# zhang-xuan1314/ABC-Net

Hardware: NVIDIA B200
Metric: images_per_sec_unet_fwd_decode (higher is better)
Workload: dtype bf16

## Files before the change

abcnet_b200/_lib.py:

```python
from __future__ import annotations

import ctypes as C
import os

_HERE = os.path.dirname(os.path.abspath(__file__))
LIB_PATH = os.path.join(_HERE, "libabcnet_b200.so")

EXPORTS = (
    "abc_last_error", "abc_version", "abc_device_ok", "abc_sm_count", "abc_launch_count",
    "abc_conv3x3_c1", "abc_conv3x3_c1_u8", "abc_conv3x3_cn", "abc_conv3x3_cn_wgrad", "abc_conv3x3_stem", "abc_conv_igemm", "abc_conv_wpack_bytes", "abc_decode_peaks",
    "abc_loss_partials", "abc_loss_backward", "abc_loss_partials_p8",
    "abc_bn_stats", "abc_bn_finalize", "abc_bn_act", "abc_bn_act_backward", "abc_nchw_to_p8", "abc_channel_sum",
    "abc_nchw_to_p8_ex", "abc_deinterleave2", "abc_conv_wgrad", "abc_conv3x3_c1_wgrad", "abc_conv3x3_c1_raw",
    "abc_heads_fused", "abc_heads_fused_pack_sizes", "abc_gather_pack", "abc_adam_step", "abc_adam_chunk_elems", "abc_assemble_molblocks", "abc_gather_patches", "abc_gather_patches_pooled", "abc_rasterise_targets",
    "abc_unet_wpack_bytes", "abc_unet_workspace_bytes", "abc_unet_create", "abc_unet_forward_infer", "abc_unet_destroy", "abc_unet_pack_host",
)


class AbcConvDesc(C.Structure):
    _fields_ = [
        ("in_", C.c_void_p), ("N", C.c_int), ("H", C.c_int), ("W", C.c_int),
        ("in_planes", C.c_int), ("in_plane_off", C.c_int), ("cin", C.c_int),
        ("wpack", C.c_void_p), ("bias", C.c_void_p),
        ("cout", C.c_int), ("n_tile", C.c_int), ("ntaps", C.c_int),
        ("tap_dy", C.c_int * 9), ("tap_dx", C.c_int * 9),
        ("act", C.c_int), ("out_mode", C.c_int),
        ("out", C.c_void_p), ("out_planes", C.c_int), ("out_plane_off", C.c_int),
        ("out_H", C.c_int), ("out_W", C.c_int),
        ("out_sy", C.c_int), ("out_oy", C.c_int), ("out_sx", C.c_int), ("out_ox", C.c_int),
        ("pool_out", C.c_void_p), ("pool_planes", C.c_int), ("pool_plane_off", C.c_int),
        ("k_segments", C.c_int), ("seg_tap0", C.c_int * 4), ("seg_ntaps", C.c_int * 4),
        ("row_fold", C.c_int), ("cta_pair", C.c_int), ("swap_mn", C.c_int),
        ("stat_sum", C.c_void_p), ("stat_sq", C.c_void_p), ("subpixel", C.c_int), ("k_chunk", C.c_int), ("act_fp16", C.c_int),
    ]


class AbcUNetConfig(C.Structure):
    _fields_ = [("in_channels", C.c_int), ("n_heads", C.c_int), ("heads", C.c_int * 16), ("crop_first", C.c_int), ("act_fp16", C.c_int)]


class AbcNamedTensor(C.Structure):
    _fields_ = [("name", C.c_char_p), ("data", C.c_void_p), ("numel", C.c_int64)]


class AbcAtomRec(C.Structure):
    _fields_ = [("x", C.c_uint16), ("y", C.c_uint16), ("type", C.c_uint8), ("charge", C.c_uint8),
                ("hs", C.c_uint8), ("pad", C.c_uint8)]


class AbcBondRec(C.Structure):
    _fields_ = [("x", C.c_uint16), ("y", C.c_uint16), ("omega", C.c_uint8), ("type", C.c_uint8),
                ("pad", C.c_uint16), ("rho", C.c_float)]


class AbcDecodeDesc(C.Structure):
    _fields_ = [
        ("maps", C.c_void_p * 8), ("N", C.c_int), ("H", C.c_int), ("W", C.c_int),
        ("c_type", C.c_int), ("c_charge", C.c_int), ("c_hs", C.c_int), ("n_omega", C.c_int), ("n_btype", C.c_int),
        ("thr", C.c_float), ("omega_mode", C.c_int),
        ("atoms", C.c_void_p), ("atom_cap", C.c_int),
        ("bonds", C.c_void_p), ("bond_cap", C.c_int),
        ("counts", C.c_void_p), ("p8f_mask", C.c_int), ("centre_prob", C.c_int), ("thr_omega", C.c_float),
        ("peak_pix", C.c_void_p), ("peak_cnt", C.c_void_p), ("peak_cap", C.c_int), ("sparse_mode", C.c_int),
        ("peak_off", C.c_void_p), ("pool_slots", C.c_int),
    ]


class AbcTargetsDesc(C.Structure):
    _fields_ = [
        ("N", C.c_int), ("H", C.c_int), ("W", C.c_int), ("n_omega", C.c_int), ("n_btype", C.c_int), ("c_type", C.c_int),
        ("c_charge", C.c_int), ("c_hs", C.c_int),
        ("atoms", C.c_void_p), ("atom_off", C.c_void_p), ("bonds", C.c_void_p), ("bond_rho", C.c_void_p), ("bond_off", C.c_void_p),
        ("atom_target", C.c_void_p), ("atom_type", C.c_void_p), ("atom_charge", C.c_void_p), ("atom_hs", C.c_void_p),
        ("bond_target", C.c_void_p), ("bond_type", C.c_void_p), ("bond_rho_map", C.c_void_p), ("bond_omega", C.c_void_p),
        ("f64", C.c_int), ("zero_first", C.c_int),
    ]


class AbcHeadsFusedDesc(C.Structure):
    _fields_ = [
        ("in_", C.c_void_p), ("N", C.c_int), ("H", C.c_int), ("W", C.c_int), ("in_planes", C.c_int), ("in_plane_off", C.c_int),
        ("w1pack", C.c_void_p), ("bias1", C.c_void_p), ("n_heads", C.c_int), ("cout", C.c_int * 16),
        ("w2pack", C.c_void_p), ("w2pack_bytes", C.c_int64), ("bias2", C.c_void_p), ("bias2_len", C.c_int),
        ("out", C.c_void_p * 16), ("out_mode", C.c_int * 16), ("out_planes", C.c_int * 16), ("item_slot", C.c_int * 6),
        ("act_fp16", C.c_int),
    ]


class AbcBnActDesc(C.Structure):
    _fields_ = [
        ("z", C.c_void_p), ("z_planes", C.c_int), ("z_plane_off", C.c_int),
        ("out", C.c_void_p), ("out_planes", C.c_int), ("out_plane_off", C.c_int),
        ("pool", C.c_void_p), ("pool_planes", C.c_int), ("pool_plane_off", C.c_int),
        ("N", C.c_int), ("H", C.c_int), ("W", C.c_int), ("C", C.c_int),
        ("scale", C.c_void_p), ("shift", C.c_void_p),
        ("act", C.c_int), ("drop_p", C.c_float), ("seed", C.c_uint64), ("seed_dev", C.c_void_p), ("drop_mask", C.c_void_p),
    ]


class AbcBnActBwdDesc(C.Structure):
    _fields_ = [
        ("z", C.c_void_p), ("z_planes", C.c_int), ("z_plane_off", C.c_int),
        ("dA", C.c_void_p), ("dA_planes", C.c_int), ("dA_plane_off", C.c_int),
        ("dP", C.c_void_p), ("dP_planes", C.c_int), ("dP_plane_off", C.c_int),
        ("dz", C.c_void_p), ("dz_planes", C.c_int), ("dz_plane_off", C.c_int),
        ("N", C.c_int), ("H", C.c_int), ("W", C.c_int), ("C", C.c_int),
        ("scale", C.c_void_p), ("shift", C.c_void_p), ("mean", C.c_void_p), ("invstd", C.c_void_p),
        ("act", C.c_int), ("drop_p", C.c_float), ("seed", C.c_uint64),
        ("s1", C.c_void_p), ("s2", C.c_void_p), ("seed_dev", C.c_void_p), ("gscale", C.c_void_p), ("drop_mask", C.c_void_p),
    ]


class AbcWgradDesc(C.Structure):
    _fields_ = [
        ("dz", C.c_void_p), ("dz_planes", C.c_int), ("dz_plane_off", C.c_int), ("cout", C.c_int),
        ("in_", C.c_void_p), ("in_planes", C.c_int), ("in_plane_off", C.c_int), ("cin", C.c_int),
        ("N", C.c_int), ("H", C.c_int), ("W", C.c_int),
        ("ntaps", C.c_int), ("tap_dy", C.c_int * 9), ("tap_dx", C.c_int * 9),
        ("dw", C.c_void_p), ("row_boxes", C.c_int),
    ]


class AbcLossDesc(C.Structure):
    _fields_ = [
        ("logits", C.c_void_p * 8), ("targets", C.c_void_p * 8), ("tgt_f64", C.c_int),
        ("N", C.c_int), ("H", C.c_int), ("W", C.c_int),
        ("c_type", C.c_int), ("c_charge", C.c_int), ("c_hs", C.c_int), ("n_omega", C.c_int), ("n_btype", C.c_int),
        ("type_weights", C.c_void_p), ("sums", C.c_void_p), ("scale", C.c_void_p),
        ("dlogits", C.c_void_p * 8),
    ]


class AbcLossP8Out(C.Structure):
    _fields_ = [("dz", C.c_void_p * 8), ("planes", C.c_int * 8), ("dbias", C.c_void_p * 8)]


assert C.sizeof(AbcAtomRec) == 8 and C.sizeof(AbcBondRec) == 12


def _load():
    if not os.path.exists(LIB_PATH):
        raise ImportError(
            f"{LIB_PATH} not found: the abcnet_b200 CUDA library has not been built "
            "(run __graft_entry__.build() or `make -C abcnet_b200/csrc`). There is no CPU fallback.")
    lib = C.CDLL(LIB_PATH)
    lib.abc_last_error.restype = C.c_char_p
    lib.abc_launch_count.restype = C.c_int64
    lib.abc_conv_wpack_bytes.restype = C.c_int64
    lib.abc_conv_wpack_bytes.argtypes = [C.c_int] * 4
    lib.abc_conv3x3_c1.argtypes = [C.c_void_p, C.c_void_p, C.c_void_p, C.c_void_p, C.c_int, C.c_int, C.c_int,
                                   C.c_int, C.c_int, C.c_void_p]
    lib.abc_conv3x3_c1_u8.argtypes = lib.abc_conv3x3_c1.argtypes
    lib.abc_conv3x3_cn.argtypes = [C.c_void_p, C.c_int, C.c_void_p, C.c_void_p, C.c_void_p, C.c_int, C.c_int, C.c_int,
                                   C.c_int, C.c_int, C.c_int, C.c_void_p]
    lib.abc_conv3x3_stem.argtypes = [C.c_void_p, C.c_int, C.c_int, C.c_void_p, C.c_void_p, C.c_void_p, C.c_int, C.c_int, C.c_int,
                                     C.c_int, C.c_int, C.c_int, C.c_void_p]
    lib.abc_conv3x3_cn_wgrad.argtypes = [C.c_void_p, C.c_int, C.c_void_p, C.c_int, C.c_int, C.c_int, C.c_int, C.c_int,
                                         C.c_void_p, C.c_void_p]
    lib.abc_conv_igemm.argtypes = [C.POINTER(AbcConvDesc), C.c_void_p]
    lib.abc_decode_peaks.argtypes = [C.POINTER(AbcDecodeDesc), C.c_void_p]
    lib.abc_loss_partials.argtypes = [C.POINTER(AbcLossDesc), C.c_void_p]
    lib.abc_loss_backward.argtypes = [C.POINTER(AbcLossDesc), C.c_void_p]
    lib.abc_loss_partials_p8.argtypes = [C.POINTER(AbcLossDesc), C.POINTER(AbcLossP8Out), C.c_void_p]
    vp, ci = C.c_void_p, C.c_int
    lib.abc_bn_stats.argtypes = [vp, ci, ci, ci, ci, ci, ci, vp, vp, vp]
    lib.abc_channel_sum.argtypes = lib.abc_bn_stats.argtypes
    lib.abc_bn_finalize.argtypes = [vp, vp, ci, C.c_double, vp, vp, C.c_float, C.c_float, vp, vp, vp, vp, vp, vp, vp]
    lib.abc_bn_act.argtypes = [C.POINTER(AbcBnActDesc), vp]
    lib.abc_bn_act_backward.argtypes = [C.POINTER(AbcBnActBwdDesc), vp]
    lib.abc_nchw_to_p8.argtypes = [vp, vp, ci, ci, ci, ci, vp]
    lib.abc_nchw_to_p8_ex.argtypes = [vp, vp, ci, ci, ci, ci, ci, vp, vp, vp]
    lib.abc_deinterleave2.argtypes = [vp, ci, ci, ci, vp, ci, ci, ci, vp]
    lib.abc_conv_wgrad.argtypes = [C.POINTER(AbcWgradDesc), vp]
    lib.abc_conv3x3_c1_wgrad.argtypes = [vp, ci, vp, ci, ci, ci, ci, ci, vp, vp]
    lib.abc_conv3x3_c1_raw.argtypes = [vp, ci, vp, vp, vp, ci, ci, ci, ci, ci, vp]
    lib.abc_heads_fused.argtypes = [C.POINTER(AbcHeadsFusedDesc), vp]
    lib.abc_heads_fused_pack_sizes.argtypes = [ci, C.POINTER(C.c_int), C.POINTER(C.c_int64), C.POINTER(C.c_int)]
    lib.abc_gather_pack.argtypes = [vp, vp, vp, C.c_int64, ci, vp]
    lib.abc_adam_step.argtypes = [vp, vp, vp, vp, vp, vp, ci, vp, vp, vp]
    lib.abc_rasterise_targets.argtypes = [C.POINTER(AbcTargetsDesc), vp]
    lib.abc_gather_patches.argtypes = [vp, ci, ci, ci, ci, vp, vp, ci, vp, vp]
    lib.abc_gather_patches_pooled.argtypes = [vp, ci, ci, ci, ci, vp, vp, vp, ci, vp, vp]
    lib.abc_unet_wpack_bytes.restype = C.c_int64
    lib.abc_unet_wpack_bytes.argtypes = [C.POINTER(AbcUNetConfig)]
    lib.abc_unet_workspace_bytes.restype = C.c_int64
    lib.abc_unet_workspace_bytes.argtypes = [C.POINTER(AbcUNetConfig), ci, ci, ci]
    lib.abc_unet_create.argtypes = [C.POINTER(AbcUNetConfig), C.POINTER(AbcNamedTensor), ci, vp, C.c_int64, vp, C.POINTER(vp)]
    lib.abc_unet_forward_infer.argtypes = [vp, vp, ci, ci, ci, ci, vp, C.c_int64, C.POINTER(vp), ci, vp]
    lib.abc_unet_destroy.argtypes = [vp]
    lib.abc_unet_pack_host.argtypes = [C.POINTER(AbcUNetConfig), C.POINTER(AbcNamedTensor), ci, vp, C.c_int64, C.POINTER(C.c_int64)]
    lib.abc_assemble_molblocks.argtypes = [vp, ci, vp, ci, vp, ci, vp, vp, ci, ci, vp, C.c_int64, vp]
    return lib


lib = _load()


def check(rc: int, what: str = "abcnet_b200") -> None:
    if rc != 0:
        msg = lib.abc_last_error()
        raise RuntimeError(f"{what} failed with status {rc}: {msg.decode() if msg else ''}")


def require_device() -> None:
    if not lib.abc_device_ok():
        msg = lib.abc_last_error()
        raise RuntimeError("abcnet_b200 needs an sm_100 (B200) CUDA device and has no CPU fallback: "
                           + (msg.decode() if msg else ""))


def current_stream_ptr() -> int:
    import torch
    return torch.cuda.current_stream().cuda_stream


def launch_count() -> int:
    return int(lib.abc_launch_count())
```

abcnet_b200/csrc/common.cu:

```cuda
#include "common.cuh"

namespace abc {

static thread_local char g_err[512] = "";
std::atomic<int64_t> g_launches{0};

void set_error(const char* fmt, ...) {
  va_list ap;
  va_start(ap, fmt);
  vsnprintf(g_err, sizeof(g_err), fmt, ap);
  va_end(ap);
}

static std::atomic<int> g_dev_ok[kMaxDevices];
static std::atomic<int> g_dev_sms[kMaxDevices];

int current_device() {
  int dev = 0;
  if (cudaGetDevice(&dev) != cudaSuccess) {
    cudaGetLastError();
    return -1;
  }
  return dev;
}

int device_check() {
  const int dev = current_device();
  if (dev < 0) {
    set_error("no CUDA device available (abcnet_b200 has no CPU fallback)");
    return ABC_ERR_NO_DEVICE;
  }
  if (dev < kMaxDevices && g_dev_ok[dev].load(std::memory_order_relaxed)) return ABC_OK;
  int major = 0;
  if (cudaDeviceGetAttribute(&major, cudaDevAttrComputeCapabilityMajor, dev) != cudaSuccess || major != 10) {
    cudaGetLastError();
    set_error("device %d has compute capability major %d; the kernels are built for sm_100a only", dev, major);
    return ABC_ERR_NO_DEVICE;
  }
  if (dev < kMaxDevices) g_dev_ok[dev].store(1, std::memory_order_relaxed);
  return ABC_OK;
}

void* tensor_map_encode_fn() {
  static void* const fn = [] {
    void* ptr = nullptr;
    cudaDriverEntryPointQueryResult qres;
    if (cudaGetDriverEntryPoint("cuTensorMapEncodeTiled", &ptr, cudaEnableDefault, &qres) == cudaSuccess &&
        qres == cudaDriverEntryPointSuccess)
      return ptr;
    cudaGetLastError();
    return static_cast<void*>(nullptr);
  }();
  return fn;
}

int sm_count() {
  const int dev = current_device();
  if (dev < 0) return 0;
  if (dev < kMaxDevices) {
    const int c = g_dev_sms[dev].load(std::memory_order_relaxed);
    if (c > 0) return c;
  }
  int n = 0;
  if (cudaDeviceGetAttribute(&n, cudaDevAttrMultiProcessorCount, dev) != cudaSuccess) {
    cudaGetLastError();
    return 0;
  }
  if (dev < kMaxDevices) g_dev_sms[dev].store(n, std::memory_order_relaxed);
  return n;
}

}

extern "C" {
const char* abc_last_error(void) { return abc::g_err; }
int abc_version(void) { return 101; }
int abc_device_ok(void) { return abc::device_check() == ABC_OK ? 1 : 0; }
int abc_sm_count(void) {
  int n = abc::sm_count();
  return n > 0 ? n : ABC_ERR_NO_DEVICE;
}
int64_t abc_launch_count(void) { return abc::g_launches.load(); }
}
```

abcnet_b200/csrc/heads_fused_sm100.cu:

```cuda
#include <cuda.h>
#include <cuda_bf16.h>

#include "common.cuh"
#include "heads_split.cuh"
#include "p8_device.cuh"
#include "ptx_sm100.cuh"

namespace abc {

constexpr int kHfThreads = 384;
constexpr int kHfMaxPairs = 8, kHfMaxItems = 6;
constexpr uint32_t kHfHeader = 4096;
constexpr uint32_t kHfARow = 10 * 16, kHfAPlane = 18 * kHfARow, kHfAStage = 8 * kHfAPlane;
constexpr uint32_t kHfBBlock = 256 * 64 * 2;
constexpr uint32_t kHfSmemLimit = 232448;
constexpr int kHfNA = 2;
constexpr int kHfNB = static_cast<int>((kHfSmemLimit - kHfHeader - kHfNA * kHfAStage) / kHfBBlock);
constexpr uint32_t kHfSmem = kHfHeader + kHfNA * kHfAStage + kHfNB * kHfBBlock;
static_assert(kHfSmem <= kHfSmemLimit, "shared memory budget");

struct HfItem {
  int head_slot;
  int nc;
  int ch0;
  int w2_off;
  int bias_off;
  int slot;
};

struct HfParams {
  int N, H, W, tiles_x, tiles_y, num_tiles, in_plane_off;
  const uint8_t* w1;
  const float* bias1;
  const uint8_t* w2;
  const float* bias2;
  int pairs;
  int cta0[kHfMaxPairs + 1];
  int bias2_off[kHfMaxPairs], bias2_len[kHfMaxPairs];
  int n_items[kHfMaxPairs];
  HfItem items[kHfMaxPairs][kHfMaxItems];
  void* out[2 * kHfMaxPairs];
  int out_mode[2 * kHfMaxPairs];
  int cout[2 * kHfMaxPairs];
  int out_planes[2 * kHfMaxPairs];
  uint32_t tap16[9];
};

template <bool kF16>
__global__ void __launch_bounds__(kHfThreads, 1)
heads_fused_kernel(const __grid_constant__ CUtensorMap tmap, const __grid_constant__ HfParams p) {
  extern __shared__ __align__(1024) uint8_t smem[];
  const uint32_t sbase = smem_u32(smem);
  const int warp = static_cast<int>(warp_id_uniform());
  const int lane = threadIdx.x & 31;
  int pair = 0;
  while (pair + 1 < p.pairs && static_cast<int>(blockIdx.x) >= p.cta0[pair + 1]) ++pair;
  const int cta_rank = blockIdx.x - p.cta0[pair], cta_stride = p.cta0[pair + 1] - p.cta0[pair];

  const uint32_t bar_a_full = sbase, bar_a_empty = sbase + 8 * kHfNA;
  const uint32_t bar_b_full = sbase + 8 * 2 * kHfNA, bar_b_empty = bar_b_full + 8 * kHfNB;
  const uint32_t bar_acc_full = bar_b_empty + 8 * kHfNB;
  const uint32_t bar_acc_empty = bar_acc_full + 16;
  const uint32_t bar_hid_full = bar_acc_empty + 16;
  const uint32_t bar_c2_full = bar_hid_full + 8;
  const uint32_t bar_c2_empty = bar_c2_full + 8;
  uint32_t* tmem_slot = reinterpret_cast<uint32_t*>(smem + 512);
  HfItem* items_s = reinterpret_cast<HfItem*>(smem + 576);
  float* bias1_s = reinterpret_cast<float*>(smem + 1024);
  float* bias2_s = reinterpret_cast<float*>(smem + 2048);
  const int n_items = p.n_items[pair];

  if (threadIdx.x == 0) {
    for (int i = 0; i < kHfNA; ++i) {
      mbar_init(bar_a_full + 8 * i, 1);
      mbar_init(bar_a_empty + 8 * i, 1);
    }
    for (int i = 0; i < kHfNB; ++i) {
      mbar_init(bar_b_full + 8 * i, 1);
      mbar_init(bar_b_empty + 8 * i, 1);
    }
    for (int i = 0; i < 2; ++i) {
      mbar_init(bar_acc_full + 8 * i, 1);
      mbar_init(bar_acc_empty + 8 * i, 8);
    }
    mbar_init(bar_hid_full, 8);
    mbar_init(bar_c2_full, 1);
    mbar_init(bar_c2_empty, 8);
    fence_mbar_init();
    tma_prefetch_desc(&tmap);
  }
  if (warp == 2) tmem_alloc<512>(smem_u32(tmem_slot));
  for (int i = threadIdx.x; i < 256; i += kHfThreads) bias1_s[i] = p.bias1[pair * 256 + i];
  for (int i = threadIdx.x; i < p.bias2_len[pair]; i += kHfThreads) bias2_s[i] = p.bias2[p.bias2_off[pair] + i];
  if (threadIdx.x < n_items) items_s[threadIdx.x] = p.items[pair][threadIdx.x];
  tc_fence_before();
  __syncthreads();
  tc_fence_after();
  const uint32_t tmem_base = *reinterpret_cast<volatile uint32_t*>(tmem_slot);

  const uint32_t a_region = sbase + kHfHeader;
  const uint32_t b_region = a_region + kHfNA * kHfAStage;
  const int tiles_per_img = p.tiles_x * p.tiles_y;
  const int my_tiles = (p.num_tiles > cta_rank) ? (p.num_tiles - cta_rank + cta_stride - 1) / cta_stride : 0;

  if (warp == 0) {
    int stage = 0;
    uint32_t phase = 0;
    for (int it = 0; it < my_tiles; ++it) {
      const int g = cta_rank + it * cta_stride;
      const int n = g / tiles_per_img;
      const int rem = g - n * tiles_per_img;
      const int ty = rem / p.tiles_x, tx = rem - ty * p.tiles_x;
      for (int kc = 0; kc < 2; ++kc) {
        mbar_wait(bar_a_empty + 8 * stage, phase ^ 1);
        if (elect_one()) {
          mbar_arrive_expect_tx(bar_a_full + 8 * stage, kHfAStage);
          tma_load_4d(a_region + stage * kHfAStage, &tmap, bar_a_full + 8 * stage, (tx * 8 - 1) * 8, ty * 16 - 1,
                      p.in_plane_off + kc * 8, n);
        }
        __syncwarp();
        if (++stage == kHfNA) {
          stage = 0;
          phase ^= 1;
        }
      }
    }
  } else if (warp == 3) {
    const uint8_t* w1 = p.w1 + static_cast<size_t>(pair) * 18 * kHfBBlock;
    int stage = 0;
    uint32_t phase = 0;
    for (int it = 0; it <= my_tiles; ++it) {
      const bool has_c1 = it < my_tiles, has_c2 = it >= 1;
      if (!has_c1 && !has_c2) break;
      int next_item = 0;
      for (int slot = 0; slot < 18; ++slot) {
        if (has_c1) {
          mbar_wait(bar_b_empty + 8 * stage, phase ^ 1);
          if (elect_one()) {
            mbar_arrive_expect_tx(bar_b_full + 8 * stage, kHfBBlock);
            bulk_load_1d(b_region + stage * kHfBBlock, w1 + static_cast<size_t>(slot) * kHfBBlock, kHfBBlock, bar_b_full + 8 * stage);
          }
          __syncwarp();
          if (++stage == kHfNB) {
            stage = 0;
            phase ^= 1;
          }
        }
        if (has_c2) {
          while (next_item < n_items && (items_s[next_item].slot <= slot || !has_c1)) {
            const uint32_t bytes = static_cast<uint32_t>(items_s[next_item].nc) * 256u;
            mbar_wait(bar_b_empty + 8 * stage, phase ^ 1);
            if (elect_one()) {
              mbar_arrive_expect_tx(bar_b_full + 8 * stage, bytes);
              bulk_load_1d(b_region + stage * kHfBBlock, p.w2 + items_s[next_item].w2_off, bytes, bar_b_full + 8 * stage);
            }
            __syncwarp();
            if (++stage == kHfNB) {
              stage = 0;
              phase ^= 1;
            }
            ++next_item;
          }
        }
      }
    }
  } else if (warp == 1) {
    const uint32_t idesc1 = umma_idesc_16(128, 256, 0, 0, kF16);
    const uint64_t a_hi64 = umma_desc_hi(kHfAPlane, kHfARow);
    const uint64_t b_hi64 = umma_desc_hi(256 * 16, 128);
    const uint32_t a_hi = static_cast<uint32_t>(a_hi64 >> 32), b_hi = static_cast<uint32_t>(b_hi64 >> 32);
    const uint32_t a_lo0 = static_cast<uint32_t>(a_hi64) | (a_region >> 4);
    const uint32_t b_lo0 = static_cast<uint32_t>(b_hi64) | (b_region >> 4);
    constexpr uint32_t a_kstep = (2 * kHfAPlane) >> 4, b_kstep = (2 * 256 * 16) >> 4;
    int a_stage = 0, b_stage = 0;
    uint32_t a_phase = 0, b_phase = 0;
    uint32_t acc_empty_phase = 0, hid_full_phase = 0, c2_empty_phase = 0;
    for (int it = 0; it <= my_tiles; ++it) {
      const bool has_c1 = it < my_tiles, has_c2 = it >= 1;
      if (!has_c1 && !has_c2) break;
      const int s = it & 1, sp = s ^ 1;
      const uint32_t tmem_d = tmem_base + s * 256;
      if (has_c1) {
        mbar_wait(bar_acc_empty + 8 * s, ((acc_empty_phase >> s) & 1u) ^ 1u);
        acc_empty_phase ^= 1u << s;
        tc_fence_after();
      }
      int next_item = 0;
      uint32_t a_base = 0;
      for (int slot = 0; slot < 18; ++slot) {
        if (has_c1) {
          const int t = slot >= 9 ? slot - 9 : slot;
          if (t == 0) {
            mbar_wait(bar_a_full + 8 * a_stage, a_phase);
            tc_fence_after();
            a_base = a_lo0 + a_stage * (kHfAStage >> 4);
          }
          mbar_wait(bar_b_full + 8 * b_stage, b_phase);
          tc_fence_after();
          const uint32_t b_base = b_lo0 + b_stage * (kHfBBlock >> 4);
          const uint32_t a_tap = a_base + p.tap16[t];
          if (elect_one()) {
#pragma unroll
            for (int j = 0; j < 4; ++j)
              umma_bf16_lohi(tmem_d, a_tap + j * a_kstep, a_hi, b_base + j * b_kstep, b_hi, idesc1, (slot | j) != 0 ? 1u : 0u);
            umma_commit(bar_b_empty + 8 * b_stage);
            if (t == 8) umma_commit(bar_a_empty + 8 * a_stage);
          }
          __syncwarp();
          if (++b_stage == kHfNB) {
            b_stage = 0;
            b_phase ^= 1;
          }
          if (t == 8 && ++a_stage == kHfNA) {
            a_stage = 0;
            a_phase ^= 1;
          }
        }
        if (has_c2) {
          while (next_item < n_items && (items_s[next_item].slot <= slot || !has_c1)) {
            const HfItem item = items_s[next_item];
            if (next_item == 0) {
              mbar_wait(bar_hid_full, hid_full_phase);
              hid_full_phase ^= 1u;
            }
            mbar_wait(bar_c2_empty, c2_empty_phase ^ 1u);
            c2_empty_phase ^= 1u;
            mbar_wait(bar_b_full + 8 * b_stage, b_phase);
            tc_fence_after();
            const uint32_t idesc2 = umma_idesc_16(128, item.nc, 0, 0, kF16);
            const uint64_t w_hi64 = umma_desc_hi(static_cast<uint32_t>(item.nc) * 16, 128);
            const uint32_t w_hi = static_cast<uint32_t>(w_hi64 >> 32);
            const uint32_t w_lo = static_cast<uint32_t>(w_hi64) | ((b_region + b_stage * kHfBBlock) >> 4);
            const uint32_t a2 = tmem_base + sp * 256 + item.head_slot * 64;
            const uint32_t d2 = tmem_base + sp * 256 + 128;
            if (elect_one()) {
#pragma unroll
              for (int k = 0; k < 8; ++k)
                umma_16_ts(d2, a2 + k * 8, w_lo + k * 2 * item.nc, w_hi, idesc2, k != 0 ? 1u : 0u);
              umma_commit(bar_b_empty + 8 * b_stage);
              umma_commit(bar_c2_full);
            }
            __syncwarp();
            if (++b_stage == kHfNB) {
              b_stage = 0;
              b_phase ^= 1;
            }
            ++next_item;
          }
        }
      }
      if (has_c1) {
        if (elect_one()) umma_commit(bar_acc_full + 8 * s);
        __syncwarp();
      }
    }
  } else if (warp >= 4) {
    const int q = warp & 3;
    const int eh = (warp - 4) >> 2;
    const int m = q * 32 + lane;
    const int r = m >> 3, c = m & 7;
    const float4* bias1_4 = reinterpret_cast<const float4*>(bias1_s);
    const float4* bias2_4 = reinterpret_cast<const float4*>(bias2_s);
    const size_t plane_px = static_cast<size_t>(p.H) * p.W;
    uint32_t acc_full_phase = 0, c2_full_phase = 0;
    for (int it = 0; it < my_tiles; ++it) {
      const int g = cta_rank + it * cta_stride;
      const int n = g / tiles_per_img;
      const int rem = g - n * tiles_per_img;
      const int ty = rem / p.tiles_x, tx = rem - ty * p.tiles_x;
      const int y = ty * 16 + r, x = tx * 8 + c;
      const bool valid = (y < p.H) && (x < p.W);
      const size_t px = static_cast<size_t>(y) * p.W + x;
      const int s = it & 1;
      const uint32_t tstage = tmem_base + s * 256 + (static_cast<uint32_t>(q * 32) << 16);
      mbar_wait(bar_acc_full + 8 * s, (acc_full_phase >> s) & 1u);
      acc_full_phase ^= 1u << s;
      tc_fence_after();
#pragma unroll 1
      for (int hs = 0; hs < 2; ++hs) {
        uint32_t raw[4][16];
#pragma unroll
        for (int i = 0; i < 4; ++i) tmem_ld16(tstage + hs * 128 + eh * 64 + i * 16, raw[i]);
        tmem_ld_wait();
        if (hs == 0) {
          tc_fence_before();
          named_bar_sync(1 + q, 64);
          tc_fence_after();
        }
        uint32_t packed[32];
#pragma unroll
        for (int i = 0; i < 4; ++i) {
          float v[16];
#pragma unroll
          for (int j = 0; j < 4; ++j) {
            const float4 bb = bias1_4[hs * 32 + eh * 16 + i * 4 + j];
            const float t0 = __uint_as_float(raw[i][4 * j + 0]) + bb.x, t1 = __uint_as_float(raw[i][4 * j + 1]) + bb.y;
            const float t2 = __uint_as_float(raw[i][4 * j + 2]) + bb.z, t3 = __uint_as_float(raw[i][4 * j + 3]) + bb.w;
            v[4 * j + 0] = fmaxf(t0, 0.01f * t0);
            v[4 * j + 1] = fmaxf(t1, 0.01f * t1);
            v[4 * j + 2] = fmaxf(t2, 0.01f * t2);
            v[4 * j + 3] = fmaxf(t3, 0.01f * t3);
          }
          const uint4 u0 = pack8_act16(v, kF16), u1 = pack8_act16(v + 8, kF16);
          packed[8 * i + 0] = u0.x; packed[8 * i + 1] = u0.y; packed[8 * i + 2] = u0.z; packed[8 * i + 3] = u0.w;
          packed[8 * i + 4] = u1.x; packed[8 * i + 5] = u1.y; packed[8 * i + 6] = u1.z; packed[8 * i + 7] = u1.w;
        }
        tmem_st16(tstage + hs * 64 + eh * 32, packed);
        tmem_st16(tstage + hs * 64 + eh * 32 + 16, packed + 16);
      }
      tmem_st_wait();
      tc_fence_before();
      __syncwarp();
      if (lane == 0) mbar_arrive(bar_hid_full);
#pragma unroll 1
      for (int ii = 0; ii < n_items; ++ii) {
        const HfItem item = items_s[ii];
        const int head = 2 * pair + item.head_slot;
        mbar_wait(bar_c2_full, c2_full_phase);
        c2_full_phase ^= 1u;
        tc_fence_after();
        const int units = item.nc >> 4;
        const int cout = p.cout[head];
        const int mode = p.out_mode[head];
        uint32_t raw[16];
#pragma unroll 1
        for (int u = eh; u < units; u += 2) {
          tmem_ld16(tstage + 128 + u * 16, raw);
          tmem_ld_wait();
          const int ch0 = item.ch0 + u * 16;
          float v[16];
#pragma unroll
          for (int i = 0; i < 4; ++i) {
            const float4 bb = bias2_4[(item.bias_off >> 2) + u * 4 + i];
            v[4 * i + 0] = __uint_as_float(raw[4 * i + 0]) + bb.x;
            v[4 * i + 1] = __uint_as_float(raw[4 * i + 1]) + bb.y;
            v[4 * i + 2] = __uint_as_float(raw[4 * i + 2]) + bb.z;
            v[4 * i + 3] = __uint_as_float(raw[4 * i + 3]) + bb.w;
          }
          if (valid && ch0 < cout) {
            if (mode == 2) {
              float4* o = reinterpret_cast<float4*>(p.out[head]) +
                          2 * ((static_cast<size_t>(n) * p.out_planes[head] + (ch0 >> 3)) * plane_px + px);
              o[0] = make_float4(v[0], v[1], v[2], v[3]);
              o[1] = make_float4(v[4], v[5], v[6], v[7]);
              if (ch0 + 8 < cout) {
                o += 2 * plane_px;
                o[0] = make_float4(v[8], v[9], v[10], v[11]);
                o[1] = make_float4(v[12], v[13], v[14], v[15]);
              }
            } else {
              float* o = reinterpret_cast<float*>(p.out[head]) + (static_cast<size_t>(n) * cout + ch0) * plane_px + px;
#pragma unroll
              for (int i = 0; i < 16; ++i)
                if (ch0 + i < cout) o[i * plane_px] = v[i];
            }
          }
        }
        tc_fence_before();
        __syncwarp();
        if (lane == 0) mbar_arrive(bar_c2_empty);
      }
      if (lane == 0) mbar_arrive(bar_acc_empty + 8 * s);
    }
  }

  tc_fence_before();
  __syncthreads();
  if (warp == 2) {
    tc_fence_after();
    tmem_dealloc<512>(tmem_base);
  }
}

typedef CUresult (*HfEncodeTiledFn)(CUtensorMap*, CUtensorMapDataType, cuuint32_t, void*, const cuuint64_t*, const cuuint64_t*,
                                    const cuuint32_t*, const cuuint32_t*, CUtensorMapInterleave, CUtensorMapSwizzle,
                                    CUtensorMapL2promotion, CUtensorMapFloatOOBfill);

static HfEncodeTiledFn hf_encode_fn() { return reinterpret_cast<HfEncodeTiledFn>(tensor_map_encode_fn()); }

}

extern "C" int abc_heads_fused(const AbcHeadsFusedDesc* d, void* stream_) {
  using namespace abc;
  if (int rc = device_check()) return rc;
  ABC_REQUIRE(d != nullptr, "abc_heads_fused: null descriptor");
  ABC_REQUIRE(d->in && d->w1pack && d->bias1 && d->w2pack && d->bias2, "abc_heads_fused: null input / weights / bias");
  ABC_REQUIRE(d->N > 0 && d->H > 0 && d->W > 0, "abc_heads_fused: bad geometry N=%d H=%d W=%d", d->N, d->H, d->W);
  ABC_REQUIRE(d->in_plane_off >= 0 && d->in_plane_off + 16 <= d->in_planes, "abc_heads_fused: the trunk has 128 channels = 16 planes");
  ABC_REQUIRE(d->n_heads >= 1 && d->n_heads <= 2 * kHfMaxPairs, "abc_heads_fused: n_heads=%d (1..%d)", d->n_heads, 2 * kHfMaxPairs);
  ABC_REQUIRE((reinterpret_cast<uintptr_t>(d->in) & 15) == 0 && (reinterpret_cast<uintptr_t>(d->w1pack) & 15) == 0 &&
                  (reinterpret_cast<uintptr_t>(d->w2pack) & 15) == 0 && (reinterpret_cast<uintptr_t>(d->bias2) & 15) == 0,
              "abc_heads_fused: buffers must be 16-byte aligned");
  const int pairs = (d->n_heads + 1) / 2;
  HfParams p{};
  p.N = d->N; p.H = d->H; p.W = d->W;
  p.tiles_x = (d->W + 7) / 8;
  p.tiles_y = (d->H + 15) / 16;
  const int64_t tiles = static_cast<int64_t>(d->N) * p.tiles_x * p.tiles_y;
  ABC_REQUIRE(tiles < (1ll << 31), "abc_heads_fused: too many tiles");
  p.num_tiles = static_cast<int>(tiles);
  p.in_plane_off = d->in_plane_off;
  p.w1 = static_cast<const uint8_t*>(d->w1pack);
  p.bias1 = d->bias1;
  p.w2 = static_cast<const uint8_t*>(d->w2pack);
  p.bias2 = d->bias2;
  for (int t = 0; t < 9; ++t) p.tap16[t] = static_cast<uint32_t>((t / 3) * 10 + (t % 3));
  int w2_off = 0, bias_off_total = 0;
  for (int pr = 0; pr < pairs; ++pr) {
    int ni = 0, bias_len = 0;
    p.bias2_off[pr] = bias_off_total;
    for (int hs = 0; hs < 2; ++hs) {
      const int head = 2 * pr + hs;
      if (head >= d->n_heads) break;
      const int cout = d->cout[head];
      ABC_REQUIRE(cout >= 1 && d->out[head] != nullptr, "abc_heads_fused: head %d: cout=%d / null output", head, cout);
      ABC_REQUIRE(d->out_mode[head] == 1 || d->out_mode[head] == 2, "abc_heads_fused: head %d: out_mode must be 1 (NCHW) or 2 (planar-8)", head);
      if (d->out_mode[head] == 2)
        ABC_REQUIRE(d->out_planes[head] >= (cout + 7) / 8, "abc_heads_fused: head %d: planar output needs %d planes", head, (cout + 7) / 8);
      p.out[head] = d->out[head];
      p.out_mode[head] = d->out_mode[head];
      p.cout[head] = cout;
      p.out_planes[head] = d->out_planes[head];
      const int chunks = (cout + 127) / 128;
      for (int cidx = 0; cidx < chunks; ++cidx) {
        ABC_REQUIRE(ni < kHfMaxItems, "abc_heads_fused: pair %d needs more than %d conv2 chunks", pr, kHfMaxItems);
        const int cnt = cout - 128 * cidx < 128 ? cout - 128 * cidx : 128;
        HfItem& it = p.items[pr][ni];
        it.head_slot = hs;
        it.nc = (cnt + 15) / 16 * 16;
        it.ch0 = 128 * cidx;
        it.w2_off = w2_off;
        it.bias_off = bias_len;
        w2_off += it.nc * 256;
        bias_len += it.nc;
        ++ni;
      }
    }
    ABC_REQUIRE(bias_len <= 512, "abc_heads_fused: pair %d: %d conv2 output columns exceed the 512 supported", pr, bias_len);
    for (int i = 0; i < ni; ++i) {
      int slot = d->item_slot[i] >= 0 && d->item_slot[i] < 18 ? d->item_slot[i] : (2 + 4 * i < 17 ? 2 + 4 * i : 17);
      if (i > 0 && slot < p.items[pr][i - 1].slot) slot = p.items[pr][i - 1].slot;
      p.items[pr][i].slot = slot;
    }
    p.n_items[pr] = ni;
    p.bias2_len[pr] = bias_len;
    bias_off_total += bias_len;
  }
  ABC_REQUIRE(w2_off == d->w2pack_bytes && bias_off_total == d->bias2_len,
              "abc_heads_fused: pack sizes differ (weights %d vs %lld bytes, bias %d vs %d floats); use abc_heads_fused_pack_sizes",
              w2_off, static_cast<long long>(d->w2pack_bytes), bias_off_total, d->bias2_len);

  HfEncodeTiledFn encode = hf_encode_fn();
  if (!encode) {
    set_error("cuTensorMapEncodeTiled driver entry point not available");
    return ABC_ERR_NO_DEVICE;
  }
  CUtensorMap tmap;
  const cuuint64_t gdim[4] = {static_cast<cuuint64_t>(d->W) * 8, static_cast<cuuint64_t>(d->H),
                              static_cast<cuuint64_t>(d->in_planes), static_cast<cuuint64_t>(d->N)};
  const cuuint64_t gstride[3] = {static_cast<cuuint64_t>(d->W) * 16, static_cast<cuuint64_t>(d->W) * d->H * 16,
                                 static_cast<cuuint64_t>(d->W) * d->H * 16 * d->in_planes};
  const cuuint32_t box[4] = {80, 18, 8, 1};
  const cuuint32_t estr[4] = {1, 1, 1, 1};
  const bool f16 = d->act_fp16 != 0;
  CUresult cr = encode(&tmap, f16 ? CU_TENSOR_MAP_DATA_TYPE_FLOAT16 : CU_TENSOR_MAP_DATA_TYPE_BFLOAT16, 4, const_cast<void*>(d->in), gdim, gstride, box, estr,
                       CU_TENSOR_MAP_INTERLEAVE_NONE, CU_TENSOR_MAP_SWIZZLE_NONE, CU_TENSOR_MAP_L2_PROMOTION_L2_256B,
                       CU_TENSOR_MAP_FLOAT_OOB_FILL_NONE);
  if (cr != CUDA_SUCCESS) {
    set_error("abc_heads_fused: cuTensorMapEncodeTiled failed with CUresult %d", static_cast<int>(cr));
    return ABC_ERR_CUDA;
  }
  static PerDeviceOnce attr_once;
  ABC_CUDA(attr_once.run([] {
    cudaError_t e = cudaFuncSetAttribute(heads_fused_kernel<false>, cudaFuncAttributeMaxDynamicSharedMemorySize, kHfSmem);
    return e != cudaSuccess ? e : cudaFuncSetAttribute(heads_fused_kernel<true>, cudaFuncAttributeMaxDynamicSharedMemorySize, kHfSmem);
  }));
  int sms = sm_count();
  if (sms <= 0) sms = 148;
  int64_t cost[kHfMaxPairs];
  for (int pr = 0; pr < pairs; ++pr) {
    int nc[kHfMaxItems], channels = 0;
    for (int i = 0; i < p.n_items[pr]; ++i) nc[i] = p.items[pr][i].nc;
    for (int hs = 0; hs < 2 && 2 * pr + hs < d->n_heads; ++hs) channels += d->cout[2 * pr + hs];
    cost[pr] = hf_pair_tile_cost(p.n_items[pr], nc, channels);
  }
  int ctas[kHfMaxPairs];
  const int total = hf_split_ctas(pairs, cost, sms, p.num_tiles, ctas);
  p.pairs = pairs;
  p.cta0[0] = 0;
  for (int pr = 0; pr < pairs; ++pr) p.cta0[pr + 1] = p.cta0[pr] + ctas[pr];
  cudaStream_t st = static_cast<cudaStream_t>(stream_);
  if (f16)
    heads_fused_kernel<true><<<total, kHfThreads, kHfSmem, st>>>(tmap, p);
  else
    heads_fused_kernel<false><<<total, kHfThreads, kHfSmem, st>>>(tmap, p);
  return launch_check("heads_fused_kernel");
}

extern "C" int abc_heads_fused_pack_sizes(int n_heads, const int* cout, int64_t* w2pack_bytes, int* bias2_len) {
  using namespace abc;
  ABC_REQUIRE(n_heads >= 1 && n_heads <= 2 * kHfMaxPairs && cout && w2pack_bytes && bias2_len, "abc_heads_fused_pack_sizes: bad arguments");
  int64_t wb = 0;
  int bl = 0;
  for (int h = 0; h < n_heads; ++h) {
    ABC_REQUIRE(cout[h] >= 1, "abc_heads_fused_pack_sizes: cout[%d]=%d", h, cout[h]);
    for (int c0 = 0; c0 < cout[h]; c0 += 128) {
      const int cnt = cout[h] - c0 < 128 ? cout[h] - c0 : 128;
      const int nc = (cnt + 15) / 16 * 16;
      wb += nc * 256;
      bl += nc;
    }
  }
  *w2pack_bytes = wb;
  *bias2_len = bl;
  return ABC_OK;
}
```

abcnet_b200/unet.py:

```python
from __future__ import annotations

import ctypes as C
import os
from collections import OrderedDict

import torch
import torch.nn as nn

from . import _lib
from ._lib import AbcConvDesc, AbcHeadsFusedDesc, check, lib

BN_EPS = 1e-5
_TAPS3 = [(ky - 1, kx - 1, ky, kx) for ky in range(3) for kx in range(3)]


def _bn(c):
    return nn.BatchNorm2d(c)


def _conv_bn_pair(cin, cout):
    holder = nn.Module()
    holder.double_conv = nn.Sequential(nn.Conv2d(cin, cout, 3, padding=1), _bn(cout), nn.ReLU(inplace=True),
                                       nn.Conv2d(cout, cout, 3, padding=1), _bn(cout), nn.ReLU(inplace=True))
    return holder


def _down(cin, cout):
    holder = nn.Module()
    holder.maxpool_conv = nn.Sequential(nn.MaxPool2d(2), _conv_bn_pair(cin, cout))
    return holder


def _up(cin, cout):
    holder = nn.Module()
    holder.up = nn.ConvTranspose2d(cin, cin // 2, kernel_size=3, stride=2)
    holder.conv = _conv_bn_pair(cin, cout)
    return holder


def _head(cin, cout):
    holder = nn.Module()
    holder.conv1 = nn.Conv2d(cin, cin, 3, padding=1)
    holder.bn = _bn(cin)
    holder.conv2 = nn.Conv2d(cin, cout, 1)
    return holder


def row_fold_for(cin, cout):
    if os.environ.get("ABCNET_NO_FOLD"):
        return 1
    if cout == 16 and cin <= 32:
        return 4
    if cout == 32 and cin <= 32:
        return 2
    return 1


def k_chunk_for(cin):
    if cin == 64 and os.environ.get("ABCNET_KC64"):
        return int(os.environ["ABCNET_KC64"])
    return min(cin, 64)


def use_cta_pair(cin, ntaps, n_tile):
    if os.environ.get("ABCNET_PAIR", "0") != "1":
        return False
    return cin % 64 == 0 and n_tile % 32 == 0 and cin * ntaps * n_tile * 2 > 160 * 1024


def swap_fold_for(cin, cout, plain_output=True):
    if os.environ.get("ABCNET_NO_SWAP") or os.environ.get("ABCNET_NO_FOLD") or os.environ.get("ABCNET_NO_SWAPFOLD") or not plain_output:
        return 0
    J = {64: 2, 32: 4}.get(cout, 0)
    if J == 4 and cin > 32:
        return 0
    return J


def use_swap(pk, out_mode, dst, pool):
    if os.environ.get("ABCNET_NO_SWAP"):
        return False
    return (pk.n_tile == 128 and (pk.fold == 1 or getattr(pk, "fold_swap", False)) and not pk.pair
            and not getattr(pk, "segments", None) and out_mode == 0 and dst is not None and pool is None)


def pair_pack(w_taps, n_tiles, n_tile):
    ntaps, _, cin = w_taps.shape
    w = w_taps.view(ntaps, n_tiles, 2, n_tile // 16, 8, cin // 64, 8, 8)
    r8 = torch.arange(8, device=w_taps.device).view(8, 1)
    pos = torch.arange(8, device=w_taps.device).view(1, 8)
    src = (pos ^ r8).view(1, 1, 1, 1, 8, 1, 8, 1).expand(ntaps, n_tiles, 2, n_tile // 16, 8, cin // 64, 8, 8)
    w = torch.gather(w, 6, src)
    return w.permute(1, 5, 0, 2, 3, 4, 6, 7)


def fold_rows_swap(w_taps, bias, taps, J):
    ntaps, cout, cin = w_taps.shape
    assert ntaps == 9 and J * cout == 128 and sorted(taps) == sorted((dy, dx) for dy in (-1, 0, 1) for dx in (-1, 0, 1))
    by_off = {t: w_taps[i] for i, t in enumerate(taps)}
    out = w_taps.new_zeros(3 * (J + 2), J, cout, cin)
    for r in range(J + 2):
        for c in range(3):
            for j in range(J):
                dy = r - 1 - j
                if -1 <= dy <= 1:
                    out[r * 3 + c, j] = by_off[(dy, c - 1)]
    return out.view(3 * (J + 2), J * cout, cin), bias.view(1, cout).expand(J, cout).reshape(-1)


def fold_rows(w_taps, bias, taps, J):
    ntaps, cout, cin = w_taps.shape
    assert ntaps == 9 and cout % 16 == 0 and sorted(taps) == sorted((dy, dx) for dy in (-1, 0, 1) for dx in (-1, 0, 1))
    by_off = {t: w_taps[i] for i, t in enumerate(taps)}
    out = w_taps.new_zeros(3 * (J + 2), cout // 16, J, 16, cin)
    for r in range(J + 2):
        for c in range(3):
            for j in range(J):
                dy = r - 1 - j
                if -1 <= dy <= 1:
                    out[r * 3 + c, :, j] = by_off[(dy, c - 1)].view(cout // 16, 16, cin)
    b = bias.view(cout // 16, 1, 16).expand(cout // 16, J, 16).reshape(-1)
    return out.view(3 * (J + 2), J * cout, cin), b


class _Packed:

    def __init__(self, w_taps, bias, taps, n_tile, cout, fold=1, pair=None, fold_swap=False, kc=None, dtype=torch.bfloat16):
        self.fold, self.fold_swap = fold, bool(fold_swap) and fold > 1
        if fold > 1:
            w_taps, bias = (fold_rows_swap if fold_swap else fold_rows)(w_taps, bias, taps, fold)
            n_tile = fold * cout
        ntaps, co, cin = w_taps.shape
        kc = kc or k_chunk_for(cin)
        self.kc = kc
        n_tiles = (cout + n_tile - 1) // n_tile
        pad = n_tiles * n_tile - co
        if pad:
            w_taps = torch.cat([w_taps, w_taps.new_zeros(ntaps, pad, cin)], 1)
            bias = torch.cat([bias, bias.new_zeros(pad)])
        if pair is None:
            pair = use_cta_pair(cin, ntaps, n_tile) and fold == 1
        self.pair = bool(pair)
        if self.pair:
            w = pair_pack(w_taps, n_tiles, n_tile)
        else:
            w = w_taps.view(ntaps, n_tiles, n_tile, cin // kc, kc // 8, 8).permute(1, 3, 0, 4, 2, 5)
        self.fp16 = dtype == torch.float16
        self.w = (w.contiguous().clamp(-65504.0, 65504.0) if self.fp16 else w.contiguous()).to(dtype)
        assert self.w.numel() * 2 == lib.abc_conv_wpack_bytes(cin, co, ntaps, n_tile)
        self.bias = bias.contiguous().float()
        self.taps, self.n_tile, self.cout, self.cin = taps, n_tile, cout, cin


def _fold(conv_w, conv_b, bn):
    scale = bn.weight.detach().float() / torch.sqrt((bn.running_var.detach().float() + bn.eps).double()).float()
    w = conv_w.detach().float() * scale.view(-1, 1, 1, 1)
    b = (conv_b.detach().float() - bn.running_mean.detach().float()) * scale + bn.bias.detach().float()
    return w, b


def _default_n_tile(cin, cout):
    env = os.environ.get(f"ABCNET_NTILE_{cin}x{cout}")
    if env:
        return int(env)
    c16 = (cout + 15) // 16 * 16
    if c16 <= 128:
        return c16
    return 256 if (cout % 256 == 0 and cin >= 128) else 128


class HeadMaps(list):

    def __init__(self, heads):
        super().__init__()
        self.heads = list(heads)

    def to_nchw(self):
        out = []
        for t, h in zip(self, self.heads):
            if t.dim() == 5:
                N, P_, H, W, _ = t.shape
                t = t.permute(0, 1, 4, 2, 3).reshape(N, P_ * 8, H, W)[:, :h].contiguous()
            out.append(t)
        return out


class _LaunchTimer:

    def __init__(self, sink, name):
        self.sink, self.name = sink, name

    def __enter__(self):
        if self.sink is not None:
            self.a = torch.cuda.Event(enable_timing=True)
            self.b = torch.cuda.Event(enable_timing=True)
            self.a.record()

    def __exit__(self, *exc):
        if self.sink is not None:
            self.b.record()
            self.sink.append((self.name, self.a, self.b))
        return False


class UNet(nn.Module):
    def __init__(self, in_channels, heads=[1, 21, 5, 1, 4, 2], crop_first=True, act_dtype="bf16"):
        super().__init__()
        if act_dtype not in ("bf16", "fp16"):
            raise ValueError("act_dtype must be 'bf16' or 'fp16'")
        self.act_dtype = act_dtype
        if not (1 <= int(in_channels) <= 8):
            raise ValueError("abcnet_b200.UNet: in_channels must be in 1..8")
        self.n_channels = int(in_channels)
        self.heads = list(heads)
        self.crop_first = bool(crop_first)
        self.s = nn.Parameter(torch.randn(10) / 100)
        self.inc1 = _conv_bn_pair(in_channels, 16)
        self.inc2 = _conv_bn_pair(16, 16)
        self.down1 = _down(16, 32)
        self.down2 = _down(32, 64)
        self.inc3 = _conv_bn_pair(64, 64)
        self.down3 = _down(64, 128)
        self.down4 = _down(128, 256)
        self.down5 = _down(256, 512)
        self.up1 = _up(512, 256)
        self.up2 = _up(256, 128)
        self.up3 = _up(128, 128)
        self.dconv1 = _conv_bn_pair(128, 128)
        self.dconv2 = _conv_bn_pair(128, 128)
        self.out_modules = nn.ModuleList([_head(128, h) for h in self.heads])
        self._packed = None
        self._packed_key = None
        self._pack_gen = 0
        self._bufs = {}
        self.timing = None
        self.dropout_p = 0.2
        self.grad_buckets = None
        self.fuse_bn = True
        self._engine = None

    def load_state_dict(self, state_dict, strict=True, **kw):
        if any(k.startswith("module.") for k in state_dict):
            state_dict = OrderedDict((k[7:] if k.startswith("module.") else k, v) for k, v in state_dict.items())
        self._packed = None
        return super().load_state_dict(state_dict, strict=strict, **kw)

    def _param_key(self):
        return tuple((p.data_ptr(), p._version) for p in list(self.parameters()) + list(self.buffers()))

    def invalidate_packed(self):
        self._packed = None
        self._packed_key = None

    def train(self, mode=True):
        self.invalidate_packed()
        return super().train(mode)

    def _dc_layers(self, holder):
        seq = holder.double_conv
        return [(seq[0], seq[1]), (seq[3], seq[4])]

    @property
    def _act_torch_dtype(self):
        return torch.float16 if self.act_dtype == "fp16" else torch.bfloat16

    @torch.no_grad()
    def prepare(self, _inspect_on_cpu=False):
        dev = self.s.device
        adt = self._act_torch_dtype
        if dev.type != "cuda" and not _inspect_on_cpu:
            raise RuntimeError("abcnet_b200.UNet runs on a CUDA (sm_100) device only; call .cuda() first -- there is no CPU path")
        P = {}

        pooled = {"inc2.3", "down1.3", "inc3.3", "down3.3", "down4.3"}

        def pack3(name, conv, bn):
            w, b = _fold(conv.weight, conv.bias, bn)
            cout, cin = w.shape[:2]
            wt = torch.stack([w[:, :, ky, kx] for (_, _, ky, kx) in _TAPS3])
            js = swap_fold_for(cin, cout, name not in pooled)
            P[name] = _Packed(wt, b, [(dy, dx) for (dy, dx, _, _) in _TAPS3], _default_n_tile(cin, cout), cout,
                              fold=js or row_fold_for(cin, cout), fold_swap=bool(js), dtype=adt)

        c0, b0 = self.inc1.double_conv[0], self.inc1.double_conv[1]
        w, b = _fold(c0.weight, c0.bias, b0)
        P["inc1.0"] = (w.reshape(16, self.n_channels * 9).contiguous(), b.contiguous())
        pack3("inc1.3", self.inc1.double_conv[3], self.inc1.double_conv[4])
        for name, holder in (("inc2", self.inc2), ("down1", self.down1.maxpool_conv[1]), ("down2", self.down2.maxpool_conv[1]),
                             ("inc3", self.inc3), ("down3", self.down3.maxpool_conv[1]), ("down4", self.down4.maxpool_conv[1]),
                             ("down5", self.down5.maxpool_conv[1]), ("up1.conv", self.up1.conv), ("up2.conv", self.up2.conv),
                             ("up3.conv", self.up3.conv), ("dconv1", self.dconv1), ("dconv2", self.dconv2)):
            (ca, ba), (cb, bb) = self._dc_layers(holder)
            pack3(name + ".0", ca, ba)
            pack3(name + ".3", cb, bb)
        for name, holder in (("up1", self.up1), ("up2", self.up2), ("up3", self.up3)):
            w = holder.up.weight.detach().float()
            b = holder.up.bias.detach().float()
            cin, cout = w.shape[:2]
            P[f"{name}.up"] = self._pack_subpixel(w, b)
            for py in (0, 1):
                for px in (0, 1):
                    ys = self._phase_taps(py)
                    xs = self._phase_taps(px)
                    taps = [(dy, dx) for (ky, dy) in ys for (kx, dx) in xs]
                    wt = torch.stack([w[:, :, ky, kx].t() for (ky, dy) in ys for (kx, dx) in xs])
                    P[f"{name}.up.{py}{px}"] = _Packed(wt.contiguous(), b, taps, _default_n_tile(cin, cout), cout, dtype=adt)
        ws, bs = [], []
        for om in self.out_modules:
            w, b = _fold(om.conv1.weight, om.conv1.bias, om.bn)
            ws.append(w)
            bs.append(b)
        w = torch.cat(ws, 0)
        wt = torch.stack([w[:, :, ky, kx] for (_, _, ky, kx) in _TAPS3])
        nt = int(os.environ.get("ABCNET_NTILE_HEADS", "256"))
        P["heads.conv1"] = _Packed(wt, torch.cat(bs), [(dy, dx) for (dy, dx, _, _) in _TAPS3], nt, w.shape[0], dtype=adt)
        P["heads.conv1.plain"] = P["heads.conv1"] if not P["heads.conv1"].pair else None
        self._heads_w1 = (wt, torch.cat(bs), w.shape[0])
        self._packed_heads_ntile = nt
        for i, om in enumerate(self.out_modules):
            w2 = om.conv2.weight.detach().float().reshape(om.conv2.weight.shape[0], -1)
            h = w2.shape[0]
            n_tile = 16 if h <= 16 else (64 if h <= 64 else (128 if h <= 128 else (192 if (h + 191) // 192 * 192 <= (h + 127) // 128 * 128 else 128)))
            P[f"heads.{i}.conv2"] = _Packed(w2.unsqueeze(0).contiguous(), om.conv2.bias.detach().float(), [(0, 0)], n_tile, h, dtype=adt)
        P["heads.fused"] = self._pack_fused_heads(dev)
        self._packed = P
        self._packed_key = self._param_key()
        self._pack_gen += 1
        return self

    def _pack_fused_heads(self, dev):
        heads = self.heads
        if len(heads) > 16 or self._packed_heads_ntile != 256:
            return None
        for i in range(0, len(heads), 2):
            pair = heads[i:i + 2]
            chunks = sum((h + 127) // 128 for h in pair)
            cols = sum(sum(((min(h - c0, 128) + 15) // 16) * 16 for c0 in range(0, h, 128)) for h in pair)
            if chunks > 6 or cols > 512:
                return None
        adt = self._act_torch_dtype
        blocks, biases = [], []
        for om, h in zip(self.out_modules, heads):
            w2 = om.conv2.weight.detach().float().reshape(h, -1)
            b2 = om.conv2.bias.detach().float()
            for c0 in range(0, h, 128):
                cnt = min(h - c0, 128)
                nc = (cnt + 15) // 16 * 16
                wb = w2.new_zeros(nc, 128)
                wb[:cnt] = w2[c0:c0 + cnt]
                wb = wb.view(nc, 16, 8).permute(1, 0, 2).contiguous()
                blocks.append((wb.clamp(-65504.0, 65504.0) if adt == torch.float16 else wb).to(adt).reshape(-1))
                bb = b2.new_zeros(nc)
                bb[:cnt] = b2[c0:c0 + cnt]
                biases.append(bb)
        w2pack = torch.cat(blocks).contiguous()
        bias2 = torch.cat(biases).contiguous()
        nb, nl = C.c_int64(0), C.c_int(0)
        check(lib.abc_heads_fused_pack_sizes(len(heads), (C.c_int * len(heads))(*heads), C.byref(nb), C.byref(nl)), "abc_heads_fused_pack_sizes")
        assert w2pack.numel() * 2 == nb.value and bias2.numel() == nl.value
        return w2pack, bias2

    def _pack_subpixel(self, w, b):
        cin, cout = w.shape[:2]
        offs = sorted({(dy, dx) for py in (0, 1) for px in (0, 1) for (_, dy) in self._phase_taps(py) for (_, dx) in self._phase_taps(px)})
        wt = w.new_zeros(len(offs), 4 * cout, cin)
        for py in (0, 1):
            for px in (0, 1):
                ph = 2 * py + px
                for (ky, dy) in self._phase_taps(py):
                    for (kx, dx) in self._phase_taps(px):
                        wt[offs.index((dy, dx)), ph * cout:(ph + 1) * cout] = w[:, :, ky, kx].t()
        pk = _Packed(wt, b.repeat(4), offs, 256 if cout % 64 == 0 else 128, 4 * cout, pair=False, dtype=self._act_torch_dtype)
        pk.subpixel = cout
        return pk

    def _phase_taps(self, parity):
        if self.crop_first:
            return [(1, 0)] if parity == 0 else [(0, 1), (2, 0)]
        return [(0, 0), (2, -1)] if parity == 0 else [(1, 0)]

    def _buf(self, key, shape):
        t = self._bufs.get(key)
        dt = self._act_torch_dtype
        if t is None or tuple(t.shape) != tuple(shape) or t.device != self.s.device or t.dtype != dt:
            t = torch.empty(shape, dtype=dt, device=self.s.device)
            self._bufs[key] = t
        return t

    @staticmethod
    def _conv(pk, src, in_plane_off, dst, out_plane_off=0, act=1, pool=None, pool_plane_off=0, out_mode=0,
              out_scale=(1, 0, 1, 0), stream=0):
        d = AbcConvDesc()
        N, in_planes, H, W, _ = src.shape
        d.in_, d.N, d.H, d.W = src.data_ptr(), N, H, W
        d.in_planes, d.in_plane_off, d.cin = in_planes, in_plane_off, pk.cin
        d.wpack, d.bias = pk.w.data_ptr(), pk.bias.data_ptr()
        d.cout, d.n_tile, d.ntaps = pk.cout, pk.n_tile, len(pk.taps)
        for i, (dy, dx) in enumerate(pk.taps):
            d.tap_dy[i], d.tap_dx[i] = dy, dx
        d.row_fold, d.cta_pair = pk.fold, int(pk.pair)
        d.k_chunk = getattr(pk, "kc", 0) if getattr(pk, "kc", 0) != min(pk.cin, 64) else 0
        d.act_fp16 = int(getattr(pk, "fp16", False))
        d.subpixel = getattr(pk, "subpixel", 0)
        d.swap_mn = int(use_swap(pk, out_mode, dst, pool)) if not d.subpixel else 0
        d.act, d.out_mode = act, out_mode
        sy, oy, sx, ox = out_scale
        d.out_sy, d.out_oy, d.out_sx, d.out_ox = sy, oy, sx, ox
        if dst is not None:
            d.out = dst.data_ptr()
            if out_mode in (0, 2):
                d.out_planes, d.out_H, d.out_W = dst.shape[1], dst.shape[2], dst.shape[3]
            else:
                d.out_planes, d.out_H, d.out_W = 0, dst.shape[2], dst.shape[3]
            d.out_plane_off = out_plane_off
        else:
            d.out, d.out_H, d.out_W = None, H, W
        if pool is not None:
            d.pool_out, d.pool_planes, d.pool_plane_off = pool.data_ptr(), pool.shape[1], pool_plane_off
        check(lib.abc_conv_igemm(C.byref(d), stream), "abc_conv_igemm")

    def _timed(self, name):
        return _LaunchTimer(self.timing, name)

    def forward(self, x):
        if self.training:
            from .train import _UNetTrainFn
            return list(_UNetTrainFn.apply(self, x, *self.parameters()))
        return self.infer(x)

    def _train_engine(self):
        if self._engine is None:
            from .train import TrainEngine
            self._engine = TrainEngine(self)
        return self._engine

    @torch.no_grad()
    def trunk_and_hidden(self, x):
        k2 = self.trunk(x)
        B, _, H4, W4, _ = k2.shape
        hid = self._buf("hid", (B, 16 * len(self.heads), H4, W4, 8))
        with self._timed("heads.conv1"):
            self._conv(self._packed["heads.conv1"], k2, 0, hid, act=2, stream=_lib.current_stream_ptr())
        return k2, hid

    @torch.no_grad()
    def trunk(self, x):
        if not x.is_cuda:
            raise RuntimeError("abcnet_b200.UNet.forward needs a CUDA tensor (no CPU fallback)")
        _lib.require_device()
        if x.dim() != 4 or x.shape[1] != self.n_channels or x.shape[2] % 32 or x.shape[3] % 32:
            raise ValueError(f"expected [B,{self.n_channels},H,W] with H, W multiples of 32, got {tuple(x.shape)}")
        if self._packed is None or self._packed_key != self._param_key():
            self.prepare()
        P = self._packed
        u8 = self.n_channels == 1 and x.dtype in (torch.uint8, torch.bool)
        x = x.contiguous().view(torch.uint8) if u8 else x.contiguous().float()
        stem_flags = 1 | (2 if self.act_dtype == "fp16" else 0)

        def first(xp, wp, bp, op, B_, H_, W_, planes, off, st_):
            return lib.abc_conv3x3_stem(xp, int(u8), self.n_channels, wp, bp, op, B_, H_, W_, planes, off, stem_flags, st_)
        B, _, H, W = x.shape
        st = _lib.current_stream_ptr()

        def cv(name, *a, **k):
            with self._timed(name):
                self._conv(P[name], *a, stream=st, **k)

        a = self._buf("a", (B, 2, H, W, 8))
        b = self._buf("b", (B, 2, H, W, 8))
        w0, b0 = P["inc1.0"]
        with self._timed("inc1.0"):
            check(first(x.data_ptr(), w0.data_ptr(), b0.data_ptr(), a.data_ptr(), B, H, W, 2, 0, st), "abc_conv3x3_stem")
        cv("inc1.3", a, 0, b)
        cv("inc2.0", b, 0, a)
        p1 = self._buf("p1", (B, 2, H // 2, W // 2, 8))
        cv("inc2.3", a, 0, None, pool=p1)
        d1 = self._buf("d1", (B, 4, H // 2, W // 2, 8))
        cv("down1.0", p1, 0, d1)
        p2 = self._buf("p2", (B, 4, H // 4, W // 4, 8))
        cv("down1.3", d1, 0, None, pool=p2)
        e1 = self._buf("e1", (B, 8, H // 4, W // 4, 8))
        e2 = self._buf("e2", (B, 8, H // 4, W // 4, 8))
        cat3 = self._buf("cat3", (B, 16, H // 4, W // 4, 8))
        cv("down2.0", p2, 0, e1)
        cv("down2.3", e1, 0, e2)
        cv("inc3.0", e2, 0, e1)
        p3 = self._buf("p3", (B, 8, H // 8, W // 8, 8))
        cv("inc3.3", e1, 0, cat3, out_plane_off=0, pool=p3)
        f1 = self._buf("f1", (B, 16, H // 8, W // 8, 8))
        cat2 = self._buf("cat2", (B, 32, H // 8, W // 8, 8))
        p4 = self._buf("p4", (B, 16, H // 16, W // 16, 8))
        cv("down3.0", p3, 0, f1)
        cv("down3.3", f1, 0, cat2, out_plane_off=0, pool=p4)
        g1 = self._buf("g1", (B, 32, H // 16, W // 16, 8))
        cat1 = self._buf("cat1", (B, 64, H // 16, W // 16, 8))
        p5 = self._buf("p5", (B, 32, H // 32, W // 32, 8))
        cv("down4.0", p4, 0, g1)
        cv("down4.3", g1, 0, cat1, out_plane_off=0, pool=p5)
        h1 = self._buf("h1", (B, 64, H // 32, W // 32, 8))
        h2 = self._buf("h2", (B, 64, H // 32, W // 32, 8))
        cv("down5.0", p5, 0, h1)
        cv("down5.3", h1, 0, h2)

        merged_up = not os.environ.get("ABCNET_UP_PHASES")

        def up(name, src, cat, half_planes):
            with self._timed(name + ".up"):
                if merged_up:
                    self._conv(P[f"{name}.up"], src, 0, cat, out_plane_off=half_planes, act=0, out_scale=(2, 0, 2, 0), stream=st)
                    return
                for py in (0, 1):
                    for px in (0, 1):
                        self._conv(P[f"{name}.up.{py}{px}"], src, 0, cat, out_plane_off=half_planes, act=0,
                                   out_scale=(2, py, 2, px), stream=st)

        up("up1", h2, cat1, 32)
        i1 = self._buf("i1", (B, 32, H // 16, W // 16, 8))
        i2 = self._buf("i2", (B, 32, H // 16, W // 16, 8))
        cv("up1.conv.0", cat1, 0, i1)
        cv("up1.conv.3", i1, 0, i2)
        up("up2", i2, cat2, 16)
        j1 = self._buf("j1", (B, 16, H // 8, W // 8, 8))
        j2 = self._buf("j2", (B, 16, H // 8, W // 8, 8))
        cv("up2.conv.0", cat2, 0, j1)
        cv("up2.conv.3", j1, 0, j2)
        up("up3", j2, cat3, 8)
        k1 = self._buf("k1", (B, 16, H // 4, W // 4, 8))
        k2 = self._buf("k2", (B, 16, H // 4, W // 4, 8))
        cv("up3.conv.0", cat3, 0, k1)
        cv("up3.conv.3", k1, 0, k2)
        cv("dconv1.0", k2, 0, k1)
        cv("dconv1.3", k1, 0, k2)
        cv("dconv2.0", k2, 0, k1)
        cv("dconv2.3", k1, 0, k2)
        return k2

    @torch.no_grad()
    def infer(self, x, outs=None, layout="nchw", fused=None):
        if layout not in ("nchw", "p8f"):
            raise ValueError("layout must be 'nchw' or 'p8f'")
        p8f = layout == "p8f"
        k2 = self.trunk(x)
        B, _, H4, W4, _ = k2.shape
        st = _lib.current_stream_ptr()
        if outs is None:
            outs = HeadMaps(self.heads)
            for h in self.heads:
                shape = (B, (h + 7) // 8, H4, W4, 8) if (p8f and h > 1) else (B, h, H4, W4)
                outs.append(torch.empty(shape, dtype=torch.float32, device=k2.device))
        fpack = self._packed.get("heads.fused")
        if fused is None:
            fused = fpack is not None and os.environ.get("ABCNET_FUSED_HEADS", "1") != "0"
        if fused:
            if fpack is None:
                raise ValueError("abc_heads_fused is not available for this head list (see include/abcnet_b200.h); use fused=False")
            w2pack, bias2 = fpack
            pk1 = self._packed["heads.conv1.plain"]
            if pk1 is None:
                wt1, b1, c1 = self._heads_w1
                pk1 = self._packed["heads.conv1.plain"] = _Packed(wt1, b1, [(dy, dx) for (dy, dx, _, _) in _TAPS3], 256, c1, pair=False,
                                                                  dtype=self._act_torch_dtype)
            d = AbcHeadsFusedDesc()
            d.in_, d.N, d.H, d.W, d.in_planes, d.in_plane_off = k2.data_ptr(), B, H4, W4, k2.shape[1], 0
            d.w1pack, d.bias1, d.n_heads = pk1.w.data_ptr(), pk1.bias.data_ptr(), len(self.heads)
            d.w2pack, d.w2pack_bytes, d.bias2, d.bias2_len = w2pack.data_ptr(), w2pack.numel() * 2, bias2.data_ptr(), bias2.numel()
            slots = [int(v) for v in os.environ.get("ABCNET_HF_SLOTS", "").split(",") if v.strip()]
            for i in range(6):
                d.item_slot[i] = slots[i] if i < len(slots) else -1
            d.act_fp16 = int(pk1.fp16)
            for i, h in enumerate(self.heads):
                d.cout[i], d.out[i] = h, outs[i].data_ptr()
                d.out_mode[i] = 2 if outs[i].dim() == 5 else 1
                d.out_planes[i] = outs[i].shape[1] if outs[i].dim() == 5 else 0
            with self._timed("heads.fused"):
                check(lib.abc_heads_fused(C.byref(d), st), "abc_heads_fused")
            return outs
        hid = self._buf("hid", (B, 16 * len(self.heads), H4, W4, 8))
        with self._timed("heads.conv1"):
            self._conv(self._packed["heads.conv1"], k2, 0, hid, act=2, stream=st)
        with self._timed("heads.conv2"):
            for i, h in enumerate(self.heads):
                self._conv(self._packed[f"heads.{i}.conv2"], hid, 16 * i, outs[i], act=0,
                           out_mode=2 if outs[i].dim() == 5 else 1, stream=st)
        return outs

    def activation(self, name):
        t = self._bufs[name]
        N, P_, H, W, _ = t.shape
        return t.float().permute(0, 1, 4, 2, 3).reshape(N, P_ * 8, H, W)
```

include/abcnet_b200.h:

```cpp
#ifndef ABCNET_B200_H_
#define ABCNET_B200_H_

#include <stdint.h>

#ifdef __cplusplus
extern "C" {
#endif

#define ABC_API __attribute__((visibility("default")))

typedef enum AbcStatus {
  ABC_OK = 0,
  ABC_ERR_INVALID = -1,
  ABC_ERR_NO_DEVICE = -2,
  ABC_ERR_CUDA = -3,
  ABC_ERR_CAPACITY = -4
} AbcStatus;

ABC_API const char* abc_last_error(void);
ABC_API int abc_version(void);
ABC_API int abc_device_ok(void);
ABC_API int abc_sm_count(void);
ABC_API int64_t abc_launch_count(void);

ABC_API int abc_conv3x3_c1(const float* img, const float* w, const float* b, void* out, int N, int H, int W,
                           int out_planes, int out_plane_off, void* stream);
ABC_API int abc_conv3x3_c1_u8(const uint8_t* img, const float* w, const float* b, void* out, int N, int H, int W,
                              int out_planes, int out_plane_off, void* stream);
ABC_API int abc_conv3x3_stem(const void* img, int img_is_u8, int cin, const float* w, const float* b, void* out, int N, int H, int W,
                             int out_planes, int out_plane_off, int flags, void* stream);
ABC_API int abc_conv3x3_cn(const float* img, int cin, const float* w, const float* b, void* out, int N, int H, int W,
                           int out_planes, int out_plane_off, int relu, void* stream);

typedef struct AbcConvDesc {
  const void* in;
  int N, H, W;
  int in_planes;
  int in_plane_off;
  int cin;
  const void* wpack;
  const float* bias;
  int cout;
  int n_tile;
  int ntaps;
  int tap_dy[9];
  int tap_dx[9];
  int act;
  int out_mode;
  void* out;
  int out_planes;
  int out_plane_off;
  int out_H, out_W;
  int out_sy, out_oy, out_sx, out_ox;
  void* pool_out;
  int pool_planes, pool_plane_off;
  int k_segments;
  int seg_tap0[4];
  int seg_ntaps[4];
  int row_fold;
  int cta_pair;
  int swap_mn;
  double* stat_sum;
  double* stat_sq;
  int subpixel;
  int k_chunk;
  int act_fp16;
} AbcConvDesc;

ABC_API int abc_conv_igemm(const AbcConvDesc* desc, void* stream);
ABC_API int64_t abc_conv_wpack_bytes(int cin, int cout, int ntaps, int n_tile);

typedef struct AbcHeadsFusedDesc {
  const void* in;
  int N, H, W;
  int in_planes, in_plane_off;
  const void* w1pack;
  const float* bias1;
  int n_heads;
  int cout[16];
  const void* w2pack;
  int64_t w2pack_bytes;
  const float* bias2;
  int bias2_len;
  void* out[16];
  int out_mode[16];
  int out_planes[16];
  int item_slot[6];
  int act_fp16;
} AbcHeadsFusedDesc;
ABC_API int abc_heads_fused(const AbcHeadsFusedDesc* desc, void* stream);
ABC_API int abc_heads_fused_pack_sizes(int n_heads, const int* cout, int64_t* w2pack_bytes, int* bias2_len);

typedef struct AbcAtomRec {
  uint16_t x, y;
  uint8_t type, charge, hs, pad;
} AbcAtomRec;
typedef struct AbcBondRec {
  uint16_t x, y;
  uint8_t omega, type;
  uint16_t pad;
  float rho;
} AbcBondRec;
typedef struct AbcDecodeDesc {
  const float* maps[8];
  int N, H, W;
  int c_type, c_charge, c_hs, n_omega, n_btype;
  float thr;
  int omega_mode;
  AbcAtomRec* atoms;
  int atom_cap;
  AbcBondRec* bonds;
  int bond_cap;
  int32_t* counts;
  int p8f_mask;
  int centre_prob;
  float thr_omega;
  int32_t* peak_pix;
  int32_t* peak_cnt;
  int peak_cap;
  int sparse_mode;
  int32_t* peak_off;
  int pool_slots;
} AbcDecodeDesc;
ABC_API int abc_decode_peaks(const AbcDecodeDesc* desc, void* stream);
ABC_API int abc_gather_patches(const void* trunk, int N, int H, int W, int planes, const int32_t* peak_pix, const int32_t* peak_cnt,
                               int peak_cap, void* out, void* stream);
ABC_API int abc_gather_patches_pooled(const void* trunk, int N, int H, int W, int planes, const int32_t* peak_pix,
                                      const int32_t* peak_cnt, const int32_t* peak_off, int pool_slots, void* out, void* stream);

ABC_API int abc_assemble_molblocks(const AbcAtomRec* atoms, int atom_cap, const AbcBondRec* bonds, int bond_cap,
                                   const int32_t* counts, int N, const double* cos_tab, const double* sin_tab, int n_omega,
                                   int n_threads, char* text, int64_t text_stride, int32_t* text_len);

typedef struct AbcLossDesc {
  const float* logits[8];
  const void* targets[8];
  int tgt_f64;
  int N, H, W;
  int c_type, c_charge, c_hs, n_omega, n_btype;
  const float* type_weights;
  double* sums;
  const float* scale;
  float* dlogits[8];
} AbcLossDesc;
enum AbcLossIndex { ABC_L_ATOM = 0, ABC_L_BOND, ABC_L_TYPE, ABC_L_CHARGE, ABC_L_BTYPE, ABC_L_RHO, ABC_L_OMEGA, ABC_L_HS };
ABC_API int abc_loss_partials(const AbcLossDesc* desc, void* stream);
ABC_API int abc_loss_backward(const AbcLossDesc* desc, void* stream);
typedef struct AbcLossP8Out {
  void* dz[8];
  int planes[8];
  double* dbias[8];
} AbcLossP8Out;
ABC_API int abc_loss_partials_p8(const AbcLossDesc* desc, const AbcLossP8Out* out, void* stream);

ABC_API int abc_bn_stats(const void* z, int N, int H, int W, int planes, int plane_off, int C, double* sum, double* sumsq, void* stream);
ABC_API int abc_bn_finalize(const double* sum, const double* sumsq, int C, double count, const float* gamma, const float* beta,
                            float eps, float momentum, float* running_mean, float* running_var, float* scale, float* shift,
                            float* mean, float* invstd, void* stream);
typedef struct AbcBnActDesc {
  const void* z; int z_planes, z_plane_off;
  void* out; int out_planes, out_plane_off;
  void* pool; int pool_planes, pool_plane_off;
  int N, H, W, C;
  const float* scale; const float* shift;
  int act;
  float drop_p; uint64_t seed;
  const uint64_t* seed_dev;
  void* drop_mask;
} AbcBnActDesc;
ABC_API int abc_bn_act(const AbcBnActDesc* desc, void* stream);
typedef struct AbcBnActBwdDesc {
  const void* z; int z_planes, z_plane_off;
  const void* dA; int dA_planes, dA_plane_off;
  const void* dP; int dP_planes, dP_plane_off;
  void* dz; int dz_planes, dz_plane_off;
  int N, H, W, C;
  const float* scale; const float* shift; const float* mean; const float* invstd;
  int act; float drop_p; uint64_t seed;
  double* s1; double* s2;
  const uint64_t* seed_dev;
  const float* gscale;
  const void* drop_mask;
} AbcBnActBwdDesc;
ABC_API int abc_bn_act_backward(const AbcBnActBwdDesc* desc, void* stream);
ABC_API int abc_nchw_to_p8(const float* src, void* dst, int N, int C, int H, int W, void* stream);
ABC_API int abc_nchw_to_p8_ex(const float* src, void* dst, int N, int C, int H, int W, int dst_planes, const float* scale,
                              double* dbias, void* stream);
ABC_API int abc_channel_sum(const void* x, int N, int H, int W, int planes, int plane_off, int C, double* sum, double* scratch, void* stream);
ABC_API int abc_deinterleave2(const void* src, int src_planes, int src_plane_off, int C, void* dst, int N, int H, int W, void* stream);
typedef struct AbcTargetsDesc {
  int N, H, W, n_omega, n_btype, c_type, c_charge, c_hs;
  const int32_t* atoms; const int32_t* atom_off;
  const int32_t* bonds; const double* bond_rho; const int32_t* bond_off;
  float* atom_target; float* atom_type; float* atom_charge; float* atom_hs; float* bond_target; float* bond_type;
  void* bond_rho_map; void* bond_omega;
  int f64;
  int zero_first;
} AbcTargetsDesc;
ABC_API int abc_rasterise_targets(const AbcTargetsDesc* desc, void* stream);

ABC_API int abc_gather_pack(const void* src_ptrs, const void* codes, void* out, int64_t n, int out_is_bf16, void* stream);
ABC_API int abc_adam_chunk_elems(void);
ABC_API int abc_adam_step(const void* p_ptrs, const void* g_ptrs, const void* m_ptrs, const void* v_ptrs, const int64_t* sizes,
                          const int32_t* chunks, int n_chunks, const float* hyper, float* step_dev, void* stream);
typedef struct AbcWgradDesc {
  const void* dz; int dz_planes, dz_plane_off; int cout;
  const void* in; int in_planes, in_plane_off; int cin;
  int N, H, W;
  int ntaps; int tap_dy[9]; int tap_dx[9];
  float* dw;
  int row_boxes;
} AbcWgradDesc;
ABC_API int abc_conv_wgrad(const AbcWgradDesc* desc, void* stream);
ABC_API int abc_conv3x3_c1_raw(const void* img, int img_is_u8, const float* w, const float* b, void* out, int N, int H, int W,
                               int out_planes, int out_plane_off, void* stream);
ABC_API int abc_conv3x3_c1_wgrad(const void* img, int img_is_u8, const void* dz, int dz_planes, int dz_plane_off, int N, int H, int W,
                                 float* dw, void* stream);
ABC_API int abc_conv3x3_cn_wgrad(const float* img, int cin, const void* dz, int dz_planes, int dz_plane_off, int N, int H, int W,
                                 float* dw, void* stream);

typedef struct AbcUNetConfig {
  int in_channels;
  int n_heads;
  int heads[16];
  int crop_first;
  int act_fp16;
} AbcUNetConfig;
typedef struct AbcNamedTensor {
  const char* name;
  const float* data;
  int64_t numel;
} AbcNamedTensor;
typedef struct AbcUNet AbcUNet;
ABC_API int64_t abc_unet_wpack_bytes(const AbcUNetConfig* cfg);
ABC_API int64_t abc_unet_workspace_bytes(const AbcUNetConfig* cfg, int N, int H, int W);
ABC_API int abc_unet_create(const AbcUNetConfig* cfg, const AbcNamedTensor* tensors, int n_tensors, void* wpack_dev, int64_t wpack_bytes,
                            void* stream, AbcUNet** out);
ABC_API int abc_unet_forward_infer(AbcUNet* net, const void* img, int img_is_u8, int N, int H, int W, void* workspace,
                                   int64_t workspace_bytes, void* const* out_ptrs, int logits_layout, void* stream);
ABC_API int abc_unet_destroy(AbcUNet* net);
ABC_API int abc_unet_pack_host(const AbcUNetConfig* cfg, const AbcNamedTensor* tensors, int n_tensors, void* out, int64_t out_bytes,
                               int64_t* used);

#ifdef __cplusplus
}
#endif
#endif
```

Baseline: 9947.

## Schedule fused head tiles through a dynamic global work queue with an item ring

Replaces the static per-pair CTA split in the fused heads kernel with a persistent dynamic scheduler. A producer warp pulls (tile, pair) items from a global atomic counter and hands them to the other warps through an 8-deep smem mbarrier ring, so each CTA can mix pairs. Biases and item tables for all pairs are now kept in shared memory. The change also adds an early conv2 drain/release path, tighter default item slot spacing, and optional per-CTA tracing. In exchange it adds an atomic per item and counter-reset logic that relies on every CTA reaching the final increment.

```diff
diff --git a/abcnet_b200/_lib.py b/abcnet_b200/_lib.py
--- a/abcnet_b200/_lib.py
+++ b/abcnet_b200/_lib.py
@@ -83,7 +83,8 @@
         ("w1pack", C.c_void_p), ("bias1", C.c_void_p), ("n_heads", C.c_int), ("cout", C.c_int * 16),
         ("w2pack", C.c_void_p), ("w2pack_bytes", C.c_int64), ("bias2", C.c_void_p), ("bias2_len", C.c_int),
         ("out", C.c_void_p * 16), ("out_mode", C.c_int * 16), ("out_planes", C.c_int * 16), ("item_slot", C.c_int * 6),
-        ("act_fp16", C.c_int),
+        ("act_fp16", C.c_int), ("trace", C.c_void_p),
+        ("work_counter", C.c_void_p), ("c2_release_late", C.c_int),
     ]
 
 
diff --git a/abcnet_b200/csrc/common.cu b/abcnet_b200/csrc/common.cu
--- a/abcnet_b200/csrc/common.cu
+++ b/abcnet_b200/csrc/common.cu
@@ -74,7 +74,7 @@
 
 extern "C" {
 const char* abc_last_error(void) { return abc::g_err; }
-int abc_version(void) { return 101; }
+int abc_version(void) { return 102; }
 int abc_device_ok(void) { return abc::device_check() == ABC_OK ? 1 : 0; }
 int abc_sm_count(void) {
   int n = abc::sm_count();
diff --git a/abcnet_b200/csrc/heads_fused_sm100.cu b/abcnet_b200/csrc/heads_fused_sm100.cu
--- a/abcnet_b200/csrc/heads_fused_sm100.cu
+++ b/abcnet_b200/csrc/heads_fused_sm100.cu
@@ -10,7 +10,9 @@
 
 constexpr int kHfThreads = 384;
 constexpr int kHfMaxPairs = 8, kHfMaxItems = 6;
-constexpr uint32_t kHfHeader = 4096;
+constexpr int kHfRing = 8;
+constexpr int kHfRingReaders = 11;
+constexpr uint32_t kHfHeader = 4096 + kHfMaxPairs * 256 * 4;
 constexpr uint32_t kHfARow = 10 * 16, kHfAPlane = 18 * kHfARow, kHfAStage = 8 * kHfAPlane;
 constexpr uint32_t kHfBBlock = 256 * 64 * 2;
 constexpr uint32_t kHfSmemLimit = 232448;
@@ -18,6 +20,7 @@
 constexpr int kHfNB = static_cast<int>((kHfSmemLimit - kHfHeader - kHfNA * kHfAStage) / kHfBBlock);
 constexpr uint32_t kHfSmem = kHfHeader + kHfNA * kHfAStage + kHfNB * kHfBBlock;
 static_assert(kHfSmem <= kHfSmemLimit, "shared memory budget");
+static_assert(kHfNB == 5, "the weight ring keeps the depth of the stand-alone conv1");
 
 struct HfItem {
   int head_slot;
@@ -27,6 +30,7 @@
   int bias_off;
   int slot;
 };
+static_assert(1088 + kHfMaxPairs * kHfMaxItems * sizeof(HfItem) <= 4096, "item tables fit the header below bias1");
 
 struct HfParams {
   int N, H, W, tiles_x, tiles_y, num_tiles, in_plane_off;
@@ -36,7 +40,6 @@
   const float* bias2;
   int pairs;
   int cta0[kHfMaxPairs + 1];
-  int bias2_off[kHfMaxPairs], bias2_len[kHfMaxPairs];
   int n_items[kHfMaxPairs];
   HfItem items[kHfMaxPairs][kHfMaxItems];
   void* out[2 * kHfMaxPairs];
@@ -44,18 +47,64 @@
   int cout[2 * kHfMaxPairs];
   int out_planes[2 * kHfMaxPairs];
   uint32_t tap16[9];
+  unsigned long long* trace;
+  int* work_counter;
+  int c2_release_late;
 };
 
-template <bool kF16>
+enum HfTraceField {
+  kTrStart, kTrEnd, kTrPair, kTrTiles,
+  kTrMmaAccEmpty, kTrMmaAFull, kTrMmaBFull, kTrMmaHidFull, kTrMmaC2Empty,
+  kTrDrain, kTrDrains,
+  kTrEpiAccFull, kTrEpiC2Full,
+  kTrBEmpty, kTrAEmpty, kTrItemWait,
+  kHfTraceFields
+};
+
+__device__ __forceinline__ unsigned long long hf_globaltimer() {
+  unsigned long long t;
+  asm volatile("mov.u64 %0, %%globaltimer;" : "=l"(t));
+  return t;
+}
+template <bool kTrace>
+__device__ __forceinline__ void hf_wait(uint32_t bar, uint32_t parity, unsigned long long& cyc) {
+  if constexpr (kTrace) {
+    const long long t0 = clock64();
+    mbar_wait(bar, parity);
+    cyc += static_cast<unsigned long long>(clock64() - t0);
+  } else {
+    mbar_wait(bar, parity);
+  }
+}
+
+struct HfItemReader {
+  uint32_t full, empty;
+  const volatile int* ring;
+  int e = 0;
+  uint32_t phase = 0;
+  template <bool kTrace>
+  __device__ __forceinline__ int next(unsigned long long& cyc) {
+    hf_wait<kTrace>(full + 8 * e, phase, cyc);
+    const int item = ring[e];
+    __syncwarp();
+    if ((threadIdx.x & 31) == 0) mbar_arrive(empty + 8 * e);
+    if (++e == kHfRing) {
+      e = 0;
+      phase ^= 1;
+    }
+    return item;
+  }
+};
+
+template <bool kF16, bool kTrace>
 __global__ void __launch_bounds__(kHfThreads, 1)
 heads_fused_kernel(const __grid_constant__ CUtensorMap tmap, const __grid_constant__ HfParams p) {
   extern __shared__ __align__(1024) uint8_t smem[];
   const uint32_t sbase = smem_u32(smem);
   const int warp = static_cast<int>(warp_id_uniform());
   const int lane = threadIdx.x & 31;
-  int pair = 0;
-  while (pair + 1 < p.pairs && static_cast<int>(blockIdx.x) >= p.cta0[pair + 1]) ++pair;
-  const int cta_rank = blockIdx.x - p.cta0[pair], cta_stride = p.cta0[pair + 1] - p.cta0[pair];
+  unsigned long long tr_start = 0;
+  if constexpr (kTrace) tr_start = hf_globaltimer();
 
   const uint32_t bar_a_full = sbase, bar_a_empty = sbase + 8 * kHfNA;
   const uint32_t bar_b_full = sbase + 8 * 2 * kHfNA, bar_b_empty = bar_b_full + 8 * kHfNB;
@@ -64,11 +113,13 @@
   const uint32_t bar_hid_full = bar_acc_empty + 16;
   const uint32_t bar_c2_full = bar_hid_full + 8;
   const uint32_t bar_c2_empty = bar_c2_full + 8;
+  const uint32_t bar_item_full = sbase + 256;
+  const uint32_t bar_item_empty = bar_item_full + 8 * kHfRing;
+  int* item_ring = reinterpret_cast<int*>(smem + 448);
   uint32_t* tmem_slot = reinterpret_cast<uint32_t*>(smem + 512);
-  HfItem* items_s = reinterpret_cast<HfItem*>(smem + 576);
-  float* bias1_s = reinterpret_cast<float*>(smem + 1024);
-  float* bias2_s = reinterpret_cast<float*>(smem + 2048);
-  const int n_items = p.n_items[pair];
+  int* n_items_s = reinterpret_cast<int*>(smem + 1024);
+  HfItem* items_s = reinterpret_cast<HfItem*>(smem + 1088);
+  float* bias1_s = reinterpret_cast<float*>(smem + 4096);
 
   if (threadIdx.x == 0) {
     for (int i = 0; i < kHfNA; ++i) {
@@ -86,13 +137,17 @@
     mbar_init(bar_hid_full, 8);
     mbar_init(bar_c2_full, 1);
     mbar_init(bar_c2_empty, 8);
+    for (int i = 0; i < kHfRing; ++i) {
+      mbar_init(bar_item_full + 8 * i, 1);
+      mbar_init(bar_item_empty + 8 * i, kHfRingReaders);
+    }
     fence_mbar_init();
     tma_prefetch_desc(&tmap);
   }
   if (warp == 2) tmem_alloc<512>(smem_u32(tmem_slot));
-  for (int i = threadIdx.x; i < 256; i += kHfThreads) bias1_s[i] = p.bias1[pair * 256 + i];
-  for (int i = threadIdx.x; i < p.bias2_len[pair]; i += kHfThreads) bias2_s[i] = p.bias2[p.bias2_off[pair] + i];
-  if (threadIdx.x < n_items) items_s[threadIdx.x] = p.items[pair][threadIdx.x];
+  for (int i = threadIdx.x; i < p.pairs * 256; i += kHfThreads) bias1_s[i] = p.bias1[i];
+  for (int i = threadIdx.x; i < p.pairs * kHfMaxItems; i += kHfThreads) items_s[i] = p.items[i / kHfMaxItems][i % kHfMaxItems];
+  if (threadIdx.x < p.pairs) n_items_s[threadIdx.x] = p.n_items[threadIdx.x];
   tc_fence_before();
   __syncthreads();
   tc_fence_after();
@@ -101,18 +156,61 @@
   const uint32_t a_region = sbase + kHfHeader;
   const uint32_t b_region = a_region + kHfNA * kHfAStage;
   const int tiles_per_img = p.tiles_x * p.tiles_y;
-  const int my_tiles = (p.num_tiles > cta_rank) ? (p.num_tiles - cta_rank + cta_stride - 1) / cta_stride : 0;
-
-  if (warp == 0) {
+  HfItemReader items{bar_item_full, bar_item_empty, item_ring};
+  unsigned long long tr_item = 0;
+
+  if (warp == 2) {
+    const int num_items = p.num_tiles * p.pairs;
+    int pair = 0;
+    while (pair + 1 < p.pairs && static_cast<int>(blockIdx.x) >= p.cta0[pair + 1]) ++pair;
+    const int cta_rank = blockIdx.x - p.cta0[pair], cta_stride = p.cta0[pair + 1] - p.cta0[pair];
+    int e = 0, taken = 0;
+    uint32_t phase = 0;
+    for (int g = cta_rank;; g += cta_stride) {
+      mbar_wait(bar_item_empty + 8 * e, phase ^ 1);
+      int item;
+      if (p.work_counter) {
+        int v = 0;
+        if (lane == 0) {
+          v = atomicAdd(p.work_counter, 1);
+          if (v == num_items + static_cast<int>(gridDim.x) - 1) atomicExch(p.work_counter, 0);
+        }
+        v = __shfl_sync(0xffffffffu, v, 0);
+        item = v < num_items ? v : -1;
+      } else {
+        item = g < p.num_tiles ? g * p.pairs + pair : -1;
+      }
+      if (lane == 0) {
+        item_ring[e] = item;
+        mbar_arrive(bar_item_full + 8 * e);
+      }
+      __syncwarp();
+      if (item < 0) break;
+      ++taken;
+      if (++e == kHfRing) {
+        e = 0;
+        phase ^= 1;
+      }
+    }
+    if constexpr (kTrace) {
+      if (lane == 0) {
+        p.trace[blockIdx.x * kHfTraceFields + kTrPair] = p.work_counter ? ~0ull : static_cast<unsigned long long>(pair);
+        p.trace[blockIdx.x * kHfTraceFields + kTrTiles] = static_cast<unsigned long long>(taken);
+      }
+    }
+  } else if (warp == 0) {
     int stage = 0;
     uint32_t phase = 0;
-    for (int it = 0; it < my_tiles; ++it) {
-      const int g = cta_rank + it * cta_stride;
+    unsigned long long tr_a_empty = 0;
+    for (;;) {
+      const int item = items.next<kTrace>(tr_item);
+      if (item < 0) break;
+      const int g = item / p.pairs;
       const int n = g / tiles_per_img;
       const int rem = g - n * tiles_per_img;
       const int ty = rem / p.tiles_x, tx = rem - ty * p.tiles_x;
       for (int kc = 0; kc < 2; ++kc) {
-        mbar_wait(bar_a_empty + 8 * stage, phase ^ 1);
+        hf_wait<kTrace>(bar_a_empty + 8 * stage, phase ^ 1, tr_a_empty);
         if (elect_one()) {
           mbar_arrive_expect_tx(bar_a_full + 8 * stage, kHfAStage);
           tma_load_4d(a_region + stage * kHfAStage, &tmap, bar_a_full + 8 * stage, (tx * 8 - 1) * 8, ty * 16 - 1,
@@ -125,17 +223,24 @@
         }
       }
     }
+    if constexpr (kTrace)
+      if (lane == 0) p.trace[blockIdx.x * kHfTraceFields + kTrAEmpty] = tr_a_empty;
   } else if (warp == 3) {
-    const uint8_t* w1 = p.w1 + static_cast<size_t>(pair) * 18 * kHfBBlock;
     int stage = 0;
     uint32_t phase = 0;
-    for (int it = 0; it <= my_tiles; ++it) {
-      const bool has_c1 = it < my_tiles, has_c2 = it >= 1;
+    unsigned long long tr_b_empty = 0;
+    for (int prev_pair = -1;;) {
+      const int item = items.next<kTrace>(tr_item);
+      const int cur_pair = item < 0 ? -1 : item % p.pairs;
+      const bool has_c1 = item >= 0, has_c2 = prev_pair >= 0;
       if (!has_c1 && !has_c2) break;
+      const uint8_t* w1 = p.w1 + static_cast<size_t>(cur_pair) * 18 * kHfBBlock;
+      const HfItem* pitems = items_s + (has_c2 ? prev_pair : 0) * kHfMaxItems;
+      const int n_prev = has_c2 ? n_items_s[prev_pair] : 0;
       int next_item = 0;
       for (int slot = 0; slot < 18; ++slot) {
         if (has_c1) {
-          mbar_wait(bar_b_empty + 8 * stage, phase ^ 1);
+          hf_wait<kTrace>(bar_b_empty + 8 * stage, phase ^ 1, tr_b_empty);
           if (elect_one()) {
             mbar_arrive_expect_tx(bar_b_full + 8 * stage, kHfBBlock);
             bulk_load_1d(b_region + stage * kHfBBlock, w1 + static_cast<size_t>(slot) * kHfBBlock, kHfBBlock, bar_b_full + 8 * stage);
@@ -146,24 +251,26 @@
             phase ^= 1;
           }
         }
-        if (has_c2) {
-          while (next_item < n_items && (items_s[next_item].slot <= slot || !has_c1)) {
-            const uint32_t bytes = static_cast<uint32_t>(items_s[next_item].nc) * 256u;
-            mbar_wait(bar_b_empty + 8 * stage, phase ^ 1);
-            if (elect_one()) {
-              mbar_arrive_expect_tx(bar_b_full + 8 * stage, bytes);
-              bulk_load_1d(b_region + stage * kHfBBlock, p.w2 + items_s[next_item].w2_off, bytes, bar_b_full + 8 * stage);
-            }
-            __syncwarp();
-            if (++stage == kHfNB) {
-              stage = 0;
-              phase ^= 1;
-            }
-            ++next_item;
-          }
-        }
-      }
-    }
+        while (next_item < n_prev && (pitems[next_item].slot <= slot || !has_c1)) {
+          const uint32_t bytes = static_cast<uint32_t>(pitems[next_item].nc) * 256u;
+          hf_wait<kTrace>(bar_b_empty + 8 * stage, phase ^ 1, tr_b_empty);
+          if (elect_one()) {
+            mbar_arrive_expect_tx(bar_b_full + 8 * stage, bytes);
+            bulk_load_1d(b_region + stage * kHfBBlock, p.w2 + pitems[next_item].w2_off, bytes, bar_b_full + 8 * stage);
+          }
+          __syncwarp();
+          if (++stage == kHfNB) {
+            stage = 0;
+            phase ^= 1;
+          }
+          ++next_item;
+        }
+      }
+      if (!has_c1) break;
+      prev_pair = cur_pair;
+    }
+    if constexpr (kTrace)
+      if (lane == 0) p.trace[blockIdx.x * kHfTraceFields + kTrBEmpty] = tr_b_empty;
   } else if (warp == 1) {
     const uint32_t idesc1 = umma_idesc_16(128, 256, 0, 0, kF16);
     const uint64_t a_hi64 = umma_desc_hi(kHfAPlane, kHfARow);
@@ -175,13 +282,17 @@
     int a_stage = 0, b_stage = 0;
     uint32_t a_phase = 0, b_phase = 0;
     uint32_t acc_empty_phase = 0, hid_full_phase = 0, c2_empty_phase = 0;
-    for (int it = 0; it <= my_tiles; ++it) {
-      const bool has_c1 = it < my_tiles, has_c2 = it >= 1;
+    unsigned long long tr_acc_empty = 0, tr_a_full = 0, tr_b_full = 0, tr_hid_full = 0, tr_c2_empty = 0;
+    for (int it = 0, prev_pair = -1;; ++it) {
+      const int item = items.next<kTrace>(tr_item);
+      const bool has_c1 = item >= 0, has_c2 = prev_pair >= 0;
       if (!has_c1 && !has_c2) break;
+      const HfItem* pitems = items_s + (has_c2 ? prev_pair : 0) * kHfMaxItems;
+      const int n_prev = has_c2 ? n_items_s[prev_pair] : 0;
       const int s = it & 1, sp = s ^ 1;
       const uint32_t tmem_d = tmem_base + s * 256;
       if (has_c1) {
-        mbar_wait(bar_acc_empty + 8 * s, ((acc_empty_phase >> s) & 1u) ^ 1u);
+        hf_wait<kTrace>(bar_acc_empty + 8 * s, ((acc_empty_phase >> s) & 1u) ^ 1u, tr_acc_empty);
         acc_empty_phase ^= 1u << s;
         tc_fence_after();
       }
@@ -191,11 +302,11 @@
         if (has_c1) {
           const int t = slot >= 9 ? slot - 9 : slot;
           if (t == 0) {
-            mbar_wait(bar_a_full + 8 * a_stage, a_phase);
+            hf_wait<kTrace>(bar_a_full + 8 * a_stage, a_phase, tr_a_full);
             tc_fence_after();
             a_base = a_lo0 + a_stage * (kHfAStage >> 4);
           }
-          mbar_wait(bar_b_full + 8 * b_stage, b_phase);
+          hf_wait<kTrace>(bar_b_full + 8 * b_stage, b_phase, tr_b_full);
           tc_fence_after();
           const uint32_t b_base = b_lo0 + b_stage * (kHfBBlock >> 4);
           const uint32_t a_tap = a_base + p.tap16[t];
@@ -216,42 +327,51 @@
             a_phase ^= 1;
           }
         }
-        if (has_c2) {
-          while (next_item < n_items && (items_s[next_item].slot <= slot || !has_c1)) {
-            const HfItem item = items_s[next_item];
-            if (next_item == 0) {
-              mbar_wait(bar_hid_full, hid_full_phase);
-              hid_full_phase ^= 1u;
-            }
-            mbar_wait(bar_c2_empty, c2_empty_phase ^ 1u);
-            c2_empty_phase ^= 1u;
-            mbar_wait(bar_b_full + 8 * b_stage, b_phase);
-            tc_fence_after();
-            const uint32_t idesc2 = umma_idesc_16(128, item.nc, 0, 0, kF16);
-            const uint64_t w_hi64 = umma_desc_hi(static_cast<uint32_t>(item.nc) * 16, 128);
-            const uint32_t w_hi = static_cast<uint32_t>(w_hi64 >> 32);
-            const uint32_t w_lo = static_cast<uint32_t>(w_hi64) | ((b_region + b_stage * kHfBBlock) >> 4);
-            const uint32_t a2 = tmem_base + sp * 256 + item.head_slot * 64;
-            const uint32_t d2 = tmem_base + sp * 256 + 128;
-            if (elect_one()) {
-#pragma unroll
-              for (int k = 0; k < 8; ++k)
-                umma_16_ts(d2, a2 + k * 8, w_lo + k * 2 * item.nc, w_hi, idesc2, k != 0 ? 1u : 0u);
-              umma_commit(bar_b_empty + 8 * b_stage);
-              umma_commit(bar_c2_full);
-            }
-            __syncwarp();
-            if (++b_stage == kHfNB) {
-              b_stage = 0;
-              b_phase ^= 1;
-            }
-            ++next_item;
-          }
-        }
-      }
-      if (has_c1) {
-        if (elect_one()) umma_commit(bar_acc_full + 8 * s);
-        __syncwarp();
+        while (next_item < n_prev && (pitems[next_item].slot <= slot || !has_c1)) {
+          const HfItem item2 = pitems[next_item];
+          if (next_item == 0) {
+            hf_wait<kTrace>(bar_hid_full, hid_full_phase, tr_hid_full);
+            hid_full_phase ^= 1u;
+          }
+          hf_wait<kTrace>(bar_c2_empty, c2_empty_phase ^ 1u, tr_c2_empty);
+          c2_empty_phase ^= 1u;
+          hf_wait<kTrace>(bar_b_full + 8 * b_stage, b_phase, tr_b_full);
+          tc_fence_after();
+          const uint32_t idesc2 = umma_idesc_16(128, item2.nc, 0, 0, kF16);
+          const uint64_t w_hi64 = umma_desc_hi(static_cast<uint32_t>(item2.nc) * 16, 128);
+          const uint32_t w_hi = static_cast<uint32_t>(w_hi64 >> 32);
+          const uint32_t w_lo = static_cast<uint32_t>(w_hi64) | ((b_region + b_stage * kHfBBlock) >> 4);
+          const uint32_t a2 = tmem_base + sp * 256 + item2.head_slot * 64;
+          const uint32_t d2 = tmem_base + sp * 256 + 128;
+          if (elect_one()) {
+#pragma unroll
+            for (int k = 0; k < 8; ++k)
+              umma_16_ts(d2, a2 + k * 8, w_lo + k * 2 * item2.nc, w_hi, idesc2, k != 0 ? 1u : 0u);
+            umma_commit(bar_b_empty + 8 * b_stage);
+            umma_commit(bar_c2_full);
+          }
+          __syncwarp();
+          if (++b_stage == kHfNB) {
+            b_stage = 0;
+            b_phase ^= 1;
+          }
+          ++next_item;
+        }
+      }
+      if (!has_c1) break;
+      if (elect_one()) umma_commit(bar_acc_full + 8 * s);
+      __syncwarp();
+      prev_pair = item % p.pairs;
+    }
+    if constexpr (kTrace) {
+      if (lane == 0) {
+        unsigned long long* tr = p.trace + blockIdx.x * kHfTraceFields;
+        tr[kTrMmaAccEmpty] = tr_acc_empty;
+        tr[kTrMmaAFull] = tr_a_full;
+        tr[kTrMmaBFull] = tr_b_full;
+        tr[kTrMmaHidFull] = tr_hid_full;
+        tr[kTrMmaC2Empty] = tr_c2_empty;
+        tr[kTrItemWait] = tr_item;
       }
     }
   } else if (warp >= 4) {
@@ -259,12 +379,14 @@
     const int eh = (warp - 4) >> 2;
     const int m = q * 32 + lane;
     const int r = m >> 3, c = m & 7;
-    const float4* bias1_4 = reinterpret_cast<const float4*>(bias1_s);
-    const float4* bias2_4 = reinterpret_cast<const float4*>(bias2_s);
     const size_t plane_px = static_cast<size_t>(p.H) * p.W;
     uint32_t acc_full_phase = 0, c2_full_phase = 0;
-    for (int it = 0; it < my_tiles; ++it) {
-      const int g = cta_rank + it * cta_stride;
+    unsigned long long tr_acc_full = 0, tr_c2_full = 0, tr_drain = 0, tr_drains = 0;
+    for (int it = 0;; ++it) {
+      const int item = items.next<kTrace>(tr_item);
+      if (item < 0) break;
+      const int g = item / p.pairs;
+      const int pair = item - g * p.pairs;
       const int n = g / tiles_per_img;
       const int rem = g - n * tiles_per_img;
       const int ty = rem / p.tiles_x, tx = rem - ty * p.tiles_x;
@@ -273,7 +395,8 @@
       const size_t px = static_cast<size_t>(y) * p.W + x;
       const int s = it & 1;
       const uint32_t tstage = tmem_base + s * 256 + (static_cast<uint32_t>(q * 32) << 16);
-      mbar_wait(bar_acc_full + 8 * s, (acc_full_phase >> s) & 1u);
+      const float4* bias1_4 = reinterpret_cast<const float4*>(bias1_s + pair * 256);
+      hf_wait<kTrace>(bar_acc_full + 8 * s, (acc_full_phase >> s) & 1u, tr_acc_full);
       acc_full_phase ^= 1u << s;
       tc_fence_after();
 #pragma unroll 1
@@ -312,55 +435,87 @@
       tc_fence_before();
       __syncwarp();
       if (lane == 0) mbar_arrive(bar_hid_full);
+      const int n_cur = n_items_s[pair];
+      const HfItem* citems = items_s + pair * kHfMaxItems;
 #pragma unroll 1
-      for (int ii = 0; ii < n_items; ++ii) {
-        const HfItem item = items_s[ii];
-        const int head = 2 * pair + item.head_slot;
-        mbar_wait(bar_c2_full, c2_full_phase);
+      for (int ii = 0; ii < n_cur; ++ii) {
+        const HfItem item2 = citems[ii];
+        const int head = 2 * pair + item2.head_slot;
+        hf_wait<kTrace>(bar_c2_full, c2_full_phase, tr_c2_full);
         c2_full_phase ^= 1u;
+        long long tr_t0 = 0;
+        if constexpr (kTrace) tr_t0 = clock64();
         tc_fence_after();
-        const int units = item.nc >> 4;
+        const int units = item2.nc >> 4;
         const int cout = p.cout[head];
         const int mode = p.out_mode[head];
-        uint32_t raw[16];
+        const bool last = ii + 1 == n_cur;
+        bool held = true;
+        auto release = [&] {
+          tc_fence_before();
+          __syncwarp();
+          if (lane == 0) {
+            mbar_arrive(bar_c2_empty);
+            if (last) mbar_arrive(bar_acc_empty + 8 * s);
+          }
+          if constexpr (kTrace) tr_drain += static_cast<unsigned long long>(clock64() - tr_t0);
+          held = false;
+        };
 #pragma unroll 1
-        for (int u = eh; u < units; u += 2) {
-          tmem_ld16(tstage + 128 + u * 16, raw);
+        for (int u0 = eh; u0 < units; u0 += 4) {
+          uint32_t raw[2][16];
+#pragma unroll
+          for (int k = 0; k < 2; ++k)
+            if (u0 + 2 * k < units) tmem_ld16(tstage + 128 + (u0 + 2 * k) * 16, raw[k]);
           tmem_ld_wait();
-          const int ch0 = item.ch0 + u * 16;
-          float v[16];
-#pragma unroll
-          for (int i = 0; i < 4; ++i) {
-            const float4 bb = bias2_4[(item.bias_off >> 2) + u * 4 + i];
-            v[4 * i + 0] = __uint_as_float(raw[4 * i + 0]) + bb.x;
-            v[4 * i + 1] = __uint_as_float(raw[4 * i + 1]) + bb.y;
-            v[4 * i + 2] = __uint_as_float(raw[4 * i + 2]) + bb.z;
-            v[4 * i + 3] = __uint_as_float(raw[4 * i + 3]) + bb.w;
-          }
-          if (valid && ch0 < cout) {
-            if (mode == 2) {
-              float4* o = reinterpret_cast<float4*>(p.out[head]) +
-                          2 * ((static_cast<size_t>(n) * p.out_planes[head] + (ch0 >> 3)) * plane_px + px);
-              o[0] = make_float4(v[0], v[1], v[2], v[3]);
-              o[1] = make_float4(v[4], v[5], v[6], v[7]);
-              if (ch0 + 8 < cout) {
-                o += 2 * plane_px;
-                o[0] = make_float4(v[8], v[9], v[10], v[11]);
-                o[1] = make_float4(v[12], v[13], v[14], v[15]);
+          if (!p.c2_release_late && u0 + 4 >= units) release();
+#pragma unroll
+          for (int k = 0; k < 2; ++k) {
+            const int u = u0 + 2 * k;
+            if (u >= units) break;
+            const int ch0 = item2.ch0 + u * 16;
+            const float4* bias2_4 = reinterpret_cast<const float4*>(p.bias2 + item2.bias_off) + u * 4;
+            float v[16];
+#pragma unroll
+            for (int i = 0; i < 4; ++i) {
+              const float4 bb = __ldg(bias2_4 + i);
+              v[4 * i + 0] = __uint_as_float(raw[k][4 * i + 0]) + bb.x;
+              v[4 * i + 1] = __uint_as_float(raw[k][4 * i + 1]) + bb.y;
+              v[4 * i + 2] = __uint_as_float(raw[k][4 * i + 2]) + bb.z;
+              v[4 * i + 3] = __uint_as_float(raw[k][4 * i + 3]) + bb.w;
+            }
+            if (valid && ch0 < cout) {
+              if (mode == 2) {
+                float4* o = reinterpret_cast<float4*>(p.out[head]) +
+                            2 * ((static_cast<size_t>(n) * p.out_planes[head] + (ch0 >> 3)) * plane_px + px);
+                o[0] = make_float4(v[0], v[1], v[2], v[3]);
+                o[1] = make_float4(v[4], v[5], v[6], v[7]);
+                if (ch0 + 8 < cout) {
+                  o += 2 * plane_px;
+                  o[0] = make_float4(v[8], v[9], v[10], v[11]);
+                  o[1] = make_float4(v[12], v[13], v[14], v[15]);
+                }
+              } else {
+                float* o = reinterpret_cast<float*>(p.out[head]) + (static_cast<size_t>(n) * cout + ch0) * plane_px + px;
+#pragma unroll
+                for (int i = 0; i < 16; ++i)
+                  if (ch0 + i < cout) o[i * plane_px] = v[i];
               }
-            } else {
-              float* o = reinterpret_cast<float*>(p.out[head]) + (static_cast<size_t>(n) * cout + ch0) * plane_px + px;
-#pragma unroll
-              for (int i = 0; i < 16; ++i)
-                if (ch0 + i < cout) o[i * plane_px] = v[i];
             }
           }
         }
-        tc_fence_before();
-        __syncwarp();
-        if (lane == 0) mbar_arrive(bar_c2_empty);
-      }
-      if (lane == 0) mbar_arrive(bar_acc_empty + 8 * s);
+        if (held) release();
+      }
+      tr_drains += n_cur;
+    }
+    if constexpr (kTrace) {
+      if (lane == 0) {
+        unsigned long long* tr = p.trace + blockIdx.x * kHfTraceFields;
+        atomicAdd(tr + kTrEpiAccFull, tr_acc_full);
+        atomicAdd(tr + kTrEpiC2Full, tr_c2_full);
+        atomicAdd(tr + kTrDrain, tr_drain);
+        atomicAdd(tr + kTrDrains, tr_drains);
+      }
     }
   }
 
@@ -369,6 +524,13 @@
   if (warp == 2) {
     tc_fence_after();
     tmem_dealloc<512>(tmem_base);
+  }
+  if constexpr (kTrace) {
+    if (threadIdx.x == 0) {
+      unsigned long long* tr = p.trace + blockIdx.x * kHfTraceFields;
+      tr[kTrStart] = tr_start;
+      tr[kTrEnd] = hf_globaltimer();
+    }
   }
 }
 
@@ -397,7 +559,7 @@
   p.tiles_x = (d->W + 7) / 8;
   p.tiles_y = (d->H + 15) / 16;
   const int64_t tiles = static_cast<int64_t>(d->N) * p.tiles_x * p.tiles_y;
-  ABC_REQUIRE(tiles < (1ll << 31), "abc_heads_fused: too many tiles");
+  ABC_REQUIRE(tiles * pairs + 1024 < (1ll << 31), "abc_heads_fused: too many tiles");
   p.num_tiles = static_cast<int>(tiles);
   p.in_plane_off = d->in_plane_off;
   p.w1 = static_cast<const uint8_t*>(d->w1pack);
@@ -408,7 +570,6 @@
   int w2_off = 0, bias_off_total = 0;
   for (int pr = 0; pr < pairs; ++pr) {
     int ni = 0, bias_len = 0;
-    p.bias2_off[pr] = bias_off_total;
     for (int hs = 0; hs < 2; ++hs) {
       const int head = 2 * pr + hs;
       if (head >= d->n_heads) break;
@@ -430,7 +591,7 @@
         it.nc = (cnt + 15) / 16 * 16;
         it.ch0 = 128 * cidx;
         it.w2_off = w2_off;
-        it.bias_off = bias_len;
+        it.bias_off = bias_off_total + bias_len;
         w2_off += it.nc * 256;
         bias_len += it.nc;
         ++ni;
@@ -438,12 +599,11 @@
     }
     ABC_REQUIRE(bias_len <= 512, "abc_heads_fused: pair %d: %d conv2 output columns exceed the 512 supported", pr, bias_len);
     for (int i = 0; i < ni; ++i) {
-      int slot = d->item_slot[i] >= 0 && d->item_slot[i] < 18 ? d->item_slot[i] : (2 + 4 * i < 17 ? 2 + 4 * i : 17);
+      int slot = d->item_slot[i] >= 0 && d->item_slot[i] < 18 ? d->item_slot[i] : (2 + 3 * i < 17 ? 2 + 3 * i : 17);
       if (i > 0 && slot < p.items[pr][i - 1].slot) slot = p.items[pr][i - 1].slot;
       p.items[pr][i].slot = slot;
     }
     p.n_items[pr] = ni;
-    p.bias2_len[pr] = bias_len;
     bias_off_total += bias_len;
   }
   ABC_REQUIRE(w2_off == d->w2pack_bytes && bias_off_total == d->bias2_len,
@@ -472,28 +632,38 @@
   }
   static PerDeviceOnce attr_once;
   ABC_CUDA(attr_once.run([] {
-    cudaError_t e = cudaFuncSetAttribute(heads_fused_kernel<false>, cudaFuncAttributeMaxDynamicSharedMemorySize, kHfSmem);
-    return e != cudaSuccess ? e : cudaFuncSetAttribute(heads_fused_kernel<true>, cudaFuncAttributeMaxDynamicSharedMemorySize, kHfSmem);
+    for (auto k : {heads_fused_kernel<false, false>, heads_fused_kernel<true, false>, heads_fused_kernel<false, true>,
+                   heads_fused_kernel<true, true>})
+      if (cudaError_t e = cudaFuncSetAttribute(k, cudaFuncAttributeMaxDynamicSharedMemorySize, kHfSmem)) return e;
+    return cudaSuccess;
   }));
   int sms = sm_count();
   if (sms <= 0) sms = 148;
-  int64_t cost[kHfMaxPairs];
-  for (int pr = 0; pr < pairs; ++pr) {
-    int nc[kHfMaxItems], channels = 0;
-    for (int i = 0; i < p.n_items[pr]; ++i) nc[i] = p.items[pr][i].nc;
-    for (int hs = 0; hs < 2 && 2 * pr + hs < d->n_heads; ++hs) channels += d->cout[2 * pr + hs];
-    cost[pr] = hf_pair_tile_cost(p.n_items[pr], nc, channels);
-  }
-  int ctas[kHfMaxPairs];
-  const int total = hf_split_ctas(pairs, cost, sms, p.num_tiles, ctas);
   p.pairs = pairs;
-  p.cta0[0] = 0;
-  for (int pr = 0; pr < pairs; ++pr) p.cta0[pr + 1] = p.cta0[pr] + ctas[pr];
+  p.work_counter = d->work_counter;
+  p.c2_release_late = d->c2_release_late != 0;
+  int total;
+  if (p.work_counter) {
+    total = static_cast<int>(tiles * pairs < sms ? tiles * pairs : sms);
+  } else {
+    int64_t cost[kHfMaxPairs];
+    for (int pr = 0; pr < pairs; ++pr) {
+      int nc[kHfMaxItems], channels = 0;
+      for (int i = 0; i < p.n_items[pr]; ++i) nc[i] = p.items[pr][i].nc;
+      for (int hs = 0; hs < 2 && 2 * pr + hs < d->n_heads; ++hs) channels += d->cout[2 * pr + hs];
+      cost[pr] = hf_pair_tile_cost(p.n_items[pr], nc, channels);
+    }
+    int ctas[kHfMaxPairs];
+    total = hf_split_ctas(pairs, cost, sms, p.num_tiles, ctas);
+    p.cta0[0] = 0;
+    for (int pr = 0; pr < pairs; ++pr) p.cta0[pr + 1] = p.cta0[pr] + ctas[pr];
+  }
   cudaStream_t st = static_cast<cudaStream_t>(stream_);
-  if (f16)
-    heads_fused_kernel<true><<<total, kHfThreads, kHfSmem, st>>>(tmap, p);
-  else
-    heads_fused_kernel<false><<<total, kHfThreads, kHfSmem, st>>>(tmap, p);
+  p.trace = reinterpret_cast<unsigned long long*>(d->trace);
+  if (p.trace) ABC_CUDA(cudaMemsetAsync(p.trace, 0, sizeof(unsigned long long) * kHfTraceFields * total, st));
+  auto kernel = f16 ? (p.trace ? heads_fused_kernel<true, true> : heads_fused_kernel<true, false>)
+                    : (p.trace ? heads_fused_kernel<false, true> : heads_fused_kernel<false, false>);
+  kernel<<<total, kHfThreads, kHfSmem, st>>>(tmap, p);
   return launch_check("heads_fused_kernel");
 }
 
diff --git a/abcnet_b200/unet.py b/abcnet_b200/unet.py
--- a/abcnet_b200/unet.py
+++ b/abcnet_b200/unet.py
@@ -234,6 +234,8 @@
         self._pack_gen = 0
         self._bufs = {}
         self.timing = None
+        self._hf_counters = {}
+        self.hf_trace = None
         self.dropout_p = 0.2
         self.grad_buckets = None
         self.fuse_bn = True
@@ -568,6 +570,13 @@
             for i in range(6):
                 d.item_slot[i] = slots[i] if i < len(slots) else -1
             d.act_fp16 = int(pk1.fp16)
+            d.trace = self.hf_trace.data_ptr() if self.hf_trace is not None else None
+            if os.environ.get("ABCNET_HF_QUEUE", "1") != "0":
+                ctr = self._hf_counters.get(k2.device)
+                if ctr is None:
+                    ctr = self._hf_counters[k2.device] = torch.zeros(1, dtype=torch.int32, device=k2.device)
+                d.work_counter = ctr.data_ptr()
+            d.c2_release_late = int(os.environ.get("ABCNET_HF_FAST_DRAIN", "1") == "0")
             for i, h in enumerate(self.heads):
                 d.cout[i], d.out[i] = h, outs[i].data_ptr()
                 d.out_mode[i] = 2 if outs[i].dim() == 5 else 1
diff --git a/include/abcnet_b200.h b/include/abcnet_b200.h
--- a/include/abcnet_b200.h
+++ b/include/abcnet_b200.h
@@ -87,6 +87,9 @@
   int out_planes[16];
   int item_slot[6];
   int act_fp16;
+  uint64_t* trace;
+  int* work_counter;
+  int c2_release_late;
 } AbcHeadsFusedDesc;
 ABC_API int abc_heads_fused(const AbcHeadsFusedDesc* desc, void* stream);
 ABC_API int abc_heads_fused_pack_sizes(int n_heads, const int* cout, int64_t* w2pack_bytes, int* bias2_len);
```

Result: faster. 10240, median of 6 (+2.9%).
